# aukeschaap/ttcross

Hardware: AMD Instinct MI355X
Metric: fiber evals/s (neval / wall time of dtt_dmrgg), Ising C_64 n=51 r=32 piv=2 (d=63) (higher is better)
Workload: dtype f64; 1 GPU; Ising C_64 n=51 r=32 piv=2 (d=63); driver=test_crs_ising c 64 51 32 2, bond_groups=8, transport=none (single process), arith=exact, sweeps=16

## Files before the change

### include/ttx.h

```cpp
#ifndef TTX_H
#define TTX_H
#include <stdint.h>

#ifdef __cplusplus
extern "C" {
#endif

#define TTX_OK 0
#define TTX_EINVAL 1
#define TTX_ENODEV 2
#define TTX_EHIP 3
#define TTX_ESTATE 4

#define TTX_FUN_ISING 1
#define TTX_FUN_STDNORM 2
#define TTX_FUN_MVN 3
#define TTX_FUN_HOST 4
#define TTX_FUN_COSCOEFF 5
#define TTX_FUN_DEVICE 6
#define TTX_FUN_TRAINS 7
#define TTX_FUN_PULLBACK 8

#define TTX_ARITH_EXACT 0
#define TTX_ARITH_FAST 1
// ... 163 lines not shown
int ttx_cores_dot_dev  (ttx_engine *h, const double *a_dev, const double *b_dev, double *out );
int ttx_cores_axpby_dev(ttx_engine *h, double alpha, const double *x_dev, double beta, double *y_dev);
int ttx_cores_get      (ttx_engine *h, double *g);
int ttx_cores_set      (ttx_engine *h, const double *g);
int ttx_cores_get_dev  (ttx_engine *h, double *g_dev);
int ttx_cores_set_dev  (ttx_engine *h, const double *g_dev);
int ttx_basis_fit_batch    (ttx_engine *h, int64_t npts, const double *x, const ttx_basis *basis, const double *y, const double *w, const ttx_fit_opts *opts,
                            double *loss, double *lambda, int32_t *cg_iters, int32_t *accepted, ttx_fit_result *result);
int ttx_basis_fit_batch_dev(ttx_engine *h, int64_t npts, const double *x_dev, const ttx_basis *basis, const double *y_dev, const double *w_dev, const ttx_fit_opts *opts,
                            double *loss, double *lambda, int32_t *cg_iters, int32_t *accepted, ttx_fit_result *result);
int ttx_basis_fit_tab      (ttx_engine *h, int64_t npts, const double *phi, const double *y, const double *w, const ttx_fit_opts *opts,
                            double *loss, double *lambda, int32_t *cg_iters, int32_t *accepted, ttx_fit_result *result);
int ttx_basis_fit_tab_dev  (ttx_engine *h, int64_t npts, const double *phi_dev, const double *y_dev, const double *w_dev, const ttx_fit_opts *opts,
                            double *loss, double *lambda, int32_t *cg_iters, int32_t *accepted, ttx_fit_result *result);
int ttx_basis_fit_last     (const ttx_engine *h, double *ms_jvp, double *ms_core_grad, double *ms_value, double *ms_vector, int64_t *n_jvp, int64_t *n_core_grad, int32_t *mode_ran);

int ttx_sq_lognorm_grad     (ttx_engine *h, const double *const *md, const double *const *mo, double gvol, double coef, double *g, int32_t accumulate, int32_t mode, double *z_mant, int64_t *z_exp, double *logz);
int ttx_sq_lognorm_grad_dev (ttx_engine *h, const double *const *md, const double *const *mo, double gvol, double coef, double *g_dev, int32_t accumulate, int32_t mode, double *z_mant, int64_t *z_exp, double *logz);
int ttx_sq_lognorm_grad_last(const ttx_engine *h, double *ms_right, double *ms_left, double *ms_asm, double *flops, int32_t *mode_ran);
int ttx_sq_nll_batch    (ttx_engine *h, int64_t npts, const double *x , const ttx_basis *basis , const double *w, double gamma, const double *const *md, const double *const *mo,
                         double gvol, int32_t mode, double *nll, double *logz, double *val, double *g);
int ttx_sq_nll_batch_dev(ttx_engine *h, int64_t npts, const double *x_dev, const ttx_basis *basis, const double *w_dev, double gamma, const double *const *md, const double *const *mo,
                         double gvol, int32_t mode, double *nll, double *logz, double *val_dev, double *g_dev);

int ttx_sample(ttx_engine *h, int64_t npts, const double *u , const double *w, const int32_t *fixed, int32_t *ind, double *logq, double *val);
int ttx_sample_dev(ttx_engine *h, int64_t npts, const double *u, const double *w, const int32_t *fixed, int32_t *ind, double *logq, double *val);
int ttx_sample_last(const ttx_engine *h, double *ms_head, double *bytes_head, double *ms_draw, int64_t *nfailed);

int ttx_sample_sq    (ttx_engine *h, int64_t npts, const double *u , const double *w, const int32_t *fixed,
                      double gamma, int32_t mode, int32_t *ind, double *logq, double *val);
int ttx_sample_sq_dev(ttx_engine *h, int64_t npts, const double *u, const double *w, const int32_t *fixed,
                      double gamma, int32_t mode, int32_t *ind, double *logq, double *val);
int ttx_sample_sq_last(const ttx_engine *h, double *ms_head, double *ms_rows, double *ms_pick, double *flops, int64_t *nfailed, int32_t *mode_ran);

int ttx_sample_real    (ttx_engine *h, int64_t npts, const double *u , const double *const *nodes ,
                        const double *cond , double *x , int32_t *cell , double *logq, double *val);
int ttx_sample_real_dev(ttx_engine *h, int64_t npts, const double *u, const double *const *nodes, const double *cond, double *x, int32_t *cell, double *logq, double *val);
int ttx_sample_real_last(const ttx_engine *h, double *ms_head, double *bytes_head, double *ms_draw, int64_t *nfailed);

int ttx_sample_sq_real    (ttx_engine *h, int64_t npts, const double *u , const double *const *nodes ,
                           const double *cond , double gamma, int32_t mode, double *x , int32_t *cell ,
                           double *logq, double *val);
int ttx_sample_sq_real_dev(ttx_engine *h, int64_t npts, const double *u, const double *const *nodes, const double *cond, double gamma, int32_t mode, double *x,
                           int32_t *cell, double *logq, double *val);
int ttx_sample_sq_real_last(const ttx_engine *h, double *ms_head, double *ms_rows, double *ms_pick, double *flops, int64_t *nfailed, int32_t *mode_ran);

int ttx_rosenblatt_sq_real    (ttx_engine *h, int64_t npts, const double *x , const double *const *nodes ,
                               const double *cond , double gamma, int32_t mode, double *u , int32_t *cell ,
                               double *logq, double *val);
int ttx_rosenblatt_sq_real_dev(ttx_engine *h, int64_t npts, const double *x, const double *const *nodes, const double *cond, double gamma, int32_t mode, double *u,
                               int32_t *cell, double *logq, double *val);
int ttx_rosenblatt_sq_real_last(const ttx_engine *h, double *ms_head, double *ms_rows, double *ms_cdf, double *flops, int64_t *nfailed, int32_t *mode_ran);

#define TTX_TOPK_ABS 0
#define TTX_TOPK_MAX 1
#define TTX_TOPK_MIN 2
int ttx_topk(ttx_engine *h, int32_t K, int32_t which, const int32_t *fixed , int32_t mode,
             int32_t *nfound, int32_t *ind , double *val , double *bound);
int ttx_topk_last(const ttx_engine *h, double *ms_gram, double *ms_score, double *ms_select, double *flops, int32_t *mode_ran);

int ttx_replicate(ttx_engine *h, ttx_engine **out);

int ttx_from_tt(ttx_engine **out, int32_t d, const int32_t *n, const int32_t *r, const double *cores, int32_t device);
int ttx_write(const ttx_engine *h, const char *path);
int ttx_read(ttx_engine **out, const char *path, int32_t device);
int ttx_get_modes(const ttx_engine *h, int32_t *d, int32_t *n);
int ttx_write_hdf5(const ttx_engine *h, const char *path);
int ttx_read_hdf5(ttx_engine **out, const char *path, int32_t device);

#define TTX_K_LOTTERY 0
#define TTX_K_HALFSTEP 1
#define TTX_K_ACCEPT 2
#define TTX_K_EXCHANGE 3
#define TTX_K_QUAD 4
#define TTX_K_OTHER 5
#define TTX_K_NKINDS 6
int ttx_set_profile(ttx_engine *h, int on);
int ttx_sweep_path(const ttx_engine *h);
int ttx_plan_describe(const ttx_engine *h, char *buf, int64_t cap);
int ttx_cluster_eval(const ttx_engine *h);
int ttx_arith(const ttx_engine *h);
int ttx_cluster_fallbacks(const ttx_engine *h);
int ttx_cluster_entry(const ttx_engine *h, int64_t out[3]);
int ttx_sweep_gap(const ttx_engine *h, int32_t out[4]);
int ttx_det_fallbacks(const ttx_engine *h);
int ttx_fun_id(const ttx_engine *h);
int64_t ttx_resid_halfsteps(const ttx_engine *h);
int ttx_kernel_stats(const ttx_engine *h, int64_t launches[TTX_K_NKINDS], double ms[TTX_K_NKINDS], double bytes[TTX_K_NKINDS]);


int ttx_k_residual_argmax(int32_t device, int32_t m, int32_t r, const double *a, const double *F, const double *x,
                          double *b_out, int32_t *imax, double *bmax);
int ttx_k_residual_bench(int32_t device, int64_t m, int32_t r, int32_t iters, double *avg_ms, double *bytes);
int ttx_k_eval(int32_t device, int32_t fun_id, int32_t d, const int32_t *n, const double *par, int32_t npar,
               const double *aux, int32_t naux, int64_t npts, const int32_t *ind, double *out);
int ttx_k_eval_arith(int32_t device, int32_t fun_id, int32_t d, const int32_t *n, const double *par, int32_t npar,
                     const double *aux, int32_t naux, int64_t npts, const int32_t *ind, double *out, int32_t arith);
int ttx_k_lottery(int32_t device, int32_t npnt, int32_t m, int32_t n, int32_t nz, const int32_t *zcol,
                  const int32_t *zrow, uint64_t rngpos, int32_t *points );
int ttx_k_fast_block(int32_t device, int32_t fun_id, int32_t d, int32_t n, const double *par, int32_t npar, const double *aux, int32_t naux,
                     int32_t p, int32_t rL, const int32_t *Lidx, int32_t rR, const int32_t *Ridx, int32_t cap, int32_t chain,
                     int64_t npts, const int32_t *pts, double *near, double *dv, double *piv, double *lot, double *colf, double *rowf,
                     double *nfar, double *pnt);
int ttx_fast_tables(const ttx_engine *h, int32_t group, int32_t side, int32_t bond, int32_t cols, int32_t *info, int32_t *idx, double *near,
                    double *dv, double *piv);

int ttx_k_exp(int32_t device, int64_t n, const double *x, double *out);
int ttx_exp_host(int64_t n, const double *x, double *out);

int ttx_k_latency_probe(int32_t device, double out[5]);

int ttx_k_rccl_selftest(int32_t device, int64_t msg_bytes, int32_t nsum);

int ttx_k_xcc_map(int32_t device, int32_t nblocks, int32_t *out);

#ifdef __cplusplus
}
#endif
#endif
```

### ttcross_amd/csrc/ttx_addr.h

```cpp
#pragma once
#include <hip/hip_runtime.h>
#include "ttx_dev.h"

__device__ __forceinline__ double *core_ptr(const DevProb &P, double *base, int g, int p, int first)
{ return base + ((size_t)g * P.NC + (p - first)) * P.CS; }
__device__ __forceinline__ double *inv_ptr(const DevProb &P, int g, int s, int first)
{ return P.inv + ((size_t)g * P.NC + (s - first + 1)) * (size_t)P.RM * P.RM; }
__device__ __forceinline__ int *vip_ptr(const DevProb &P, int g, int s, int first)
{ return P.vip + ((size_t)g * P.NC + (s - first + 1)) * (size_t)4 * P.RM; }
__device__ __forceinline__ short *L_ptr(const DevProb &P, int g, int s, int first)
{ return P.L + ((size_t)g * P.NC + (s - first + 1)) * (size_t)P.d * P.RM; }
__device__ __forceinline__ short *R_ptr(const DevProb &P, int g, int s, int first)
{ return P.R + ((size_t)g * P.NC + (s - first)) * (size_t)P.d * P.RM; }
```

### ttcross_amd/csrc/ttx_cluster.h

```cpp
#pragma once
#include "ttx_fused.h"
#include "ttx_mvn.h"
#include "ttx_cluster_rules.h"

#define CB 256

struct ClD2 { double a, b; };
struct ClStrided {
    const char *p; size_t sb; unsigned at;
    __device__ __forceinline__ ClStrided(const double *base, size_t at_, size_t stride) : p((const char *)base), sb(8 * stride), at((unsigned)(8 * at_)) {}
    __device__ __forceinline__ double operator()() { const double v = *(const double *)(p + at); p += sb; return v; }
};

__device__ __forceinline__ double f_ising_c4p(int m, int A, const double *an, const double *aw, double s1n, double s1w,
                                              double s2n, double s2w, const double *bn, const double *bw,
                                              double pv, double pvk, double pw, double pwk)
{
    const int nb = m - A - 2;
    double v = pv, w = pw, vk = pvk, wk = pwk;
    auto vstep = [&](double xv) { vk = vk * xv; v = v + vk; };
    auto wstep = [&](double xv) { wk = wk * xv; w = w + wk; };
    vstep(s2n); vstep(s1n);
    chain8v<true>(an, A, vstep);
    wstep(s1n); wstep(s2n);
// ... 47 lines not shown
}
__device__ __forceinline__ void wave_argmax2(double &a, double &v, int &idx)
{
    const double amx = wave_max_key(a);
    const int key = (a == amx && idx != INT_MAX) ? ((idx << 1) | (signbit(v) ? 1 : 0)) : INT_MAX;
    const int kmin = wave_min_i(key);
    a = amx;
    if (kmin == INT_MAX) { idx = INT_MAX; v = 0.0; }
    else { idx = kmin >> 1; v = (kmin & 1) ? -amx : amx; }
}

__device__ __forceinline__ double f_ising_cfast(double xj, double wj, double xk, double wk, double pv, double pvk, double pw, double pwk,
                                                double SL, double WL, double SR, double WR)
{
    const double v = pv + pvk * xk * (1.0 + xj * (1.0 + SL));
    const double w = pw + pwk * xj * (1.0 + xk * (1.0 + SR));
    return 2.0 / (v * w) * ((WL * wj) * (wk * WR));
}

typedef unsigned int u4 __attribute__((ext_vector_type(4)));
struct ClRec { u4 a, b; };
static_assert(sizeof(ClRec) == sizeof(ClPart), "record buffers are sized as ClPart: [2][G][TTX_CLREC] u4 arg-max records, then as many running-maximum records");
__device__ __forceinline__ void st16(void *p, u4 v) { asm volatile("global_store_dwordx4 %0, %1, off sc1" :: "v"(p), "v"(v) : "memory"); }
__device__ __forceinline__ u4 ld16(const void *p)
{
    u4 v;
    asm volatile("global_load_dwordx4 %0, %1, off sc1\n\ts_waitcnt vmcnt(0)" : "=v"(v) : "v"(p) : "memory");
    return v;
}

__device__ __forceinline__ int xcc_id() { return (int)__builtin_amdgcn_s_getreg(((4 - 1) << 11) | 20) & 15; }

__device__ __forceinline__ bool cluster_sync(unsigned *ctr, unsigned target, int *abortflag, int *s_ok)
{
    asm volatile("s_waitcnt vmcnt(0)" ::: "memory");
    __syncthreads();
    if (threadIdx.x == 0) {
        int ok = 1;
        unsigned spins = 0;
        __hip_atomic_fetch_add(ctr, 1u, __ATOMIC_RELEASE, __HIP_MEMORY_SCOPE_AGENT);
        while (__hip_atomic_load(ctr, __ATOMIC_RELAXED, __HIP_MEMORY_SCOPE_AGENT) < target) {
            __builtin_amdgcn_s_sleep(1);
            if (++spins > (1u << 22)) { ok = 0; __hip_atomic_store(abortflag, 1, __ATOMIC_RELAXED, __HIP_MEMORY_SCOPE_SYSTEM); break; }
            if ((spins & 1023u) == 0 && __hip_atomic_load(abortflag, __ATOMIC_RELAXED, __HIP_MEMORY_SCOPE_SYSTEM)) { ok = 0; break; }
        }
        __atomic_thread_fence(__ATOMIC_ACQUIRE);
        *s_ok = ok;
    }
    __syncthreads();
    return *s_ok != 0;
}

#ifdef TTX_STAMPS
#define CST_DECL const bool t_me = (threadIdx.x == 0 && g == 0 && cb == 0); long long t_prev = wall_clock64()
#define CST(k) do { if (t_me) { long long t_now = wall_clock64(); gs.stamp[0][k] += t_now - t_prev; t_prev = t_now; } } while (0)
#define CST_END() do { if (t_me) gs.nstamp[0]++; } while (0)
#define CSE_DECL const int t_eb = (threadIdx.x == 0 && g == 0 && cb <= 1) ? cb : -1; long long t_eprev = wall_clock64()
#define CSE_MARK() do { if (t_eb >= 0) t_eprev = wall_clock64(); } while (0)
#define CSE(k) do { if (t_eb >= 0) { long long t_now = wall_clock64(); P.gs[0].stamp[1][8 * t_eb + (k)] += t_now - t_eprev; t_eprev = t_now; } } while (0)
#define CSE_END() do { if (t_eb == 0) P.gs[0].nstamp[1]++; } while (0)
#define WST(k) do { if (P.dbg && g == 0 && epoch == 8 && pp == 4 && lane == 0 && h < 8) P.dbg[((size_t)(h * 64 + cb * 4 + wv)) * 8 + (k)] = (long long)__builtin_readcyclecounter(); } while (0)
#else
#define WST(k)
#define CST_DECL
#define CST(k)
#define CST_END()
#define CSE_DECL
#define CSE_MARK()
#define CSE(k)
#define CSE_END()
#endif

#define CL_ZKEEP 1
#define CL_ZCARRY 2
#define CL_WORD 4
#define CL_POWTAB 8
#define CL_PACK2 16
static_assert(CL_POWTAB_N == CB, "one table entry per thread of a workgroup");
__device__ const ClPowTab cl_powtab = cl_make_powtab();
struct ClArgs { DevProb P; int dir, nsteps, NB, ldsinv, epoch, zkeep; };
__device__ __forceinline__ int *cl_zimage(const DevProb &P, int g, int nsteps)
{ return (int *)(P.cl_part + (size_t)2 * P.G * TTX_CLREC) + (size_t)g * cl_zimage_ints(nsteps, P.RM); }

template <bool CFAST, bool CPAD>
__global__ __launch_bounds__(CB) void k_sweep_cluster(DevProb P, int dir, int nsteps, int NB, int ldsinv, int epoch, int zkeep)
{
    extern __shared__ __align__(16) double dyn[];
    __shared__ int zc[128], zr[128], zcs[128], zrs[128], keepc[128], keepr[128];
    __shared__ int nzc, nzr, nsc, nsr, s_ok;
    __shared__ int slt[2][TTX_CLMAX + 1], wtab[TTX_CLMAX];
    __shared__ ttx_cdfseg segc[TTX_TABSEG], segr[TTX_TABSEG];
    __shared__ double sha[8], shv[8], shm[8]; __shared__ int shi[8];
    __shared__ double pLw[64], pLk[64], pRv[64], pRk[64];
    static_assert(!(CFAST && CPAD), "the closed form reads the rows in dimension order");
    constexpr int NFT = CFAST ? 64 : 1;
    __shared__ double fSL[NFT], fWL[NFT], fSR[NFT], fWR[NFT];
    __shared__ struct { int ii, jj, kk, qq, hcount, rc_k, rc_q, rr_i, rr_j; double pivot, amax, bytes_half; long long neval, n_resid; } s_rook;
    const int bid = blockIdx.x;
    const int g = (bid & 7) + 8 * (bid / (8 * NB)), cb = (bid >> 3) % NB;
    CSE_DECL;
    if (g >= P.G || P.ctl[0]) return;
    const int bpar = (epoch - 1) & 1;
    if (P.tail_side && epoch >= 2) {
        const TailRec &t0 = P.tailrec[(size_t)bpar * P.G];
        if (stop_rule(epoch - 1, P.maxrank, P.accuracy, t0.pivotmax, max_pos(t0.amax, P.gs[0].amax_bnd[bpar]), P.strk[epoch & 1]).ready) return;
    }
    if (P.cl_test_abort && P.cl_test_abort == epoch && g == 0 && cb == 0) {
        if (threadIdx.x == 0) { __hip_atomic_store(P.cl_abort, 1, __ATOMIC_RELAXED, __HIP_MEMORY_SCOPE_SYSTEM); P.ctl[0] = 1; }
        return;
    }
    const int tid = threadIdx.x, m = P.d, RM = P.RM, NM = P.NM;
    const int lane = tid & 63, wv = tid >> 6;
    GroupState &gs = P.gs[g];
    const int first = gs.first, last = gs.last, nbonds = last - first + 1;
    int *r = P.r + (size_t)g * (m + 2);
    const int VS = ((m + 7) & ~7) + 8;
    const int RS = 2 * VS + 2;
    const int n1m = P.n[1];
    const int SL = RM * ((NM + NB - 1) / NB + 1);
    unsigned *ctr = P.cl_ctr + g;
    unsigned nbar = (unsigned)(epoch - 1) * (unsigned)min(nsteps, nbonds);
    ClPart *part = P.cl_part;
    double *par = dyn;
    double *XL = par + ((P.npar + 1) & ~1);
    double *XR = XL + (size_t)RM * RS;
    double *acol = XR + (size_t)RM * RS;
    double *arow = acol + SL;
    double *resc = arow + SL;
    double *resr = resc + SL;
    double *xsc = resr + SL;
    double *xsr = xsc + ((RM + 1) & ~1);
    int *lot = (int *)(xsr + ((RM + 1) & ~1));
    double *GL = (double *)(lot + 4 * ((2 * RM + 2 * NM + 4 + 1) & ~1));
    double *GU = GL + (size_t)RM * RM;
    int *ZK = (int *)(ldsinv ? GU + (size_t)RM * RM : GL);
    int *ZN = ZK + (size_t)nsteps * 2 * RM;
    for (int x = tid; x < P.npar; x += CB) par[x] = P.par[x];
    if (cb == 0) {
        if (tid == 0) { gs.pivotmax = -1.0; gs.pivotmin = -1.0; }
        int *rr = P.rr + (size_t)g * (m + 2);
        for (int s = tid; s <= m; s += CB) rr[s] = r[s];
    }
    __syncthreads();
    CSE(0);
    if ((zkeep & CL_ZCARRY) && cl_lists_valid(gs.zk_epoch, epoch)) {
        const int *img = cl_zimage(P, g, nsteps);
        for (int x = tid; x < nbonds * 2 * RM; x += CB) ZK[x] = img[x];
        for (int x = tid; x < 2 * nbonds; x += CB) ZN[x] = img[(size_t)nsteps * 2 * RM + x];
        if (cb == 0 && tid == 0) gs.n_zload++;
        __syncthreads();
    } else if (zkeep & CL_ZKEEP) {
        int *TMP = (int *)XL;
        const int E = nbonds * 2 * RM;
        for (int x = tid; x < E; x += CB) {
            const int b = x / (2 * RM), side = (x / RM) & 1, u = x % RM, pb = first + b;
            if (u < r[pb]) { const int *vp = vip_ptr(P, g, pb, first) + 4 * u; TMP[x] = (vp[2 * side + 1] << 16) | vp[2 * side]; }
        }
        __syncthreads();
        for (int x = tid; x < E; x += CB) {
            const int b = x / (2 * RM), u = x % RM, nb_ = r[first + b];
            if (u < nb_) {
                const int *src = TMP + (x - u); const int a = src[u]; int ra = 0;
                for (int t = 0; t < nb_; t++) ra += (src[t] < a) || (src[t] == a && t < u);
                ZK[(x - u) + ra] = a;
            }
        }
        __syncthreads();
        for (int x = tid; x < E; x += CB) {
            const int b = x / (2 * RM), u = x % RM, nb_ = r[first + b];
            if (u < nb_) {
                const int *src = ZK + (x - u); int pc = 0;
                for (int t = 1; t <= u; t++) pc += (src[t] != src[t - 1]);
                const bool keep = (u == 0) || (src[u] != src[u - 1]);
                TMP[x] = keep ? pc : -1;
                if (u == nb_ - 1) ZN[x / RM] = pc + 1;
            }
        }
        __syncthreads();
        int mykey = 0, mypos = -1;
        for (int x0 = 0; x0 < E; x0 += CB) {
            const int x = x0 + tid;
            mypos = -1;
            if (x < E) { const int b = x / (2 * RM), u = x % RM; if (u < r[first + b]) { mypos = TMP[x]; mykey = ZK[x]; } }
            __syncthreads();
            if (mypos >= 0) ZK[(x - x % RM) + mypos] = mykey;
            __syncthreads();
        }
    }
    double amax = gs.amax, pivotmax = -1.0, pivotmin = -1.0;
    if (P.tail_side && epoch >= 2) amax = max_pos(amax, gs.amax_bnd[bpar]);
    const double pivotmax_prev = gs.pivotmax_prev;
    long long neval = gs.neval;
    unsigned long long rngpos = gs.rngpos;
    double bytes_half = gs.bytes_half; long long n_resid = gs.n_resid;
    int hcount = 0;
    CSE(1);
    const bool ptab = (zkeep & CL_POWTAB) != 0;
    const unsigned long long bil0 = ptab ? cl_powtab.v[tid] : ttx_minstd_pow(2ull * tid);
    unsigned long long sA0;
    {
        const unsigned long long cw = gs.rngword, cwpos = gs.rngword_pos;
        if ((zkeep & CL_WORD) && cl_word_valid(cw, cwpos, rngpos)) { sA0 = cw; if (cb == 0 && tid == 0) gs.n_wload++; }
        else sA0 = ttx_minstd_pow(2 * rngpos + 1);
    }
    const int bl0 = ptab ? (int)cl_powtab.v[lane] : (int)ttx_minstd_pow(2ull * lane);
    constexpr unsigned long long c64 = cl_minstd_pow_c(128);
    CSE(2);
    CST_DECL;

    for (int pp = 1; pp <= nsteps; pp++) {
        if (pp > nbonds) break;
        const int p = (dir == 1) ? first + pp - 1 : last + 1 - pp;
        const int r0 = r[p - 1], r1 = r[p], r2 = r[p + 1], n1 = P.n[p], n2 = P.n[p + 1];
        const int nlot = r0 + n1 + n2 + r2;
        double *Cp = core_ptr(P, P.col, g, p, first), *Wq = core_ptr(P, P.row, g, p + 1, first);
        double *Ap = core_ptr(P, P.arg, g, p, first), *Aq = core_ptr(P, P.arg, g, p + 1, first);
        const short *Lt = L_ptr(P, g, p - 1, first), *Rt = R_ptr(P, g, p + 1, first);
        const int cA = (p - 1 + 7) >> 3, cB = (m - p - 1 + 7) >> 3;
        const int sside = (tid >> 6) & 1, sseg = tid & 63;
        double sg_a0 = 0.0, sg_al = 0.0, sg_de = 0.0; int sg_k0 = 0, sg_cn = 0, myns = 0;
        auto seg_issue = [&](int Kc_, int Kr_) {
            if (tid >= 128) {
                const int K = sside ? Kr_ : Kc_; const ttx_cdfseg *sp = P.cdf_tab + (size_t)K * TTX_TABSEG + sseg;
                myns = P.cdf_ns[K]; sg_a0 = sp->a0; sg_al = sp->alast; sg_de = sp->delta; sg_k0 = sp->k0; sg_cn = sp->cnt;
            }
        };
        {
            const int AL = min(VS, (p - 1 + 7) & ~7), AR = min(VS, (m - p - 1 + 7) & ~7);
            if (AL > 0) {
                int c = tid / AL, o = tid - c * AL;
                const int dc = CB / AL, dO = CB - dc * AL;
                while (c < r0) {
                    if constexpr (CPAD) {
                        if (o < p - 1) {
                            const int ix = (int)Lt[(size_t)o * RM + c];
                            XL[(size_t)c * RS + (p - 2 - o)] = par[ix - 1]; XL[(size_t)c * RS + VS + o] = par[n1m + ix - 1];
                        } else { XL[(size_t)c * RS + o] = 0.0; XL[(size_t)c * RS + VS + o] = 1.0; }
                    } else {
                        const int ix = (o < p - 1) ? (int)Lt[(size_t)o * RM + c] : 1;
                        XL[(size_t)c * RS + o] = par[ix - 1]; XL[(size_t)c * RS + VS + o] = par[n1m + ix - 1];
                    }
                    c += dc; o += dO; if (o >= AL) { o -= AL; c++; }
                }
            }
            if (AR > 0) {
                int c = tid / AR, o = tid - c * AR;
                const int dc = CB / AR, dO = CB - dc * AR;
                while (c < r2) {
                    if (CPAD && o >= m - p - 1) { XR[(size_t)c * RS + o] = 0.0; XR[(size_t)c * RS + VS + o] = 1.0; }
                    else {
                        const int ix = (o < m - p - 1) ? (int)Rt[(size_t)o * RM + c] : 1;
                        XR[(size_t)c * RS + o] = par[ix - 1]; XR[(size_t)c * RS + VS + o] = par[n1m + ix - 1];
                    }
                    c += dc; o += dO; if (o >= AR) { o -= AR; c++; }
                }
            }
        }
        if (ldsinv) {
            if (p > first) { const double *gL = inv_ptr(P, g, p - 1, first); for (int x = tid; x < r0 * r0; x += CB) GL[x] = gL[x]; }
            if (p < last)  { const double *gU = inv_ptr(P, g, p + 1, first); for (int x = tid; x < r2 * r2; x += CB) GU[x] = gU[x]; }
        }
        CST(0);
        if (zkeep & CL_ZKEEP) seg_issue(r0 * n1 - ZN[2 * (p - first)], n2 * r2 - ZN[2 * (p - first) + 1]);
        static_assert(2 * (TTX_CLMAX + 1) <= 64 && TTX_CLMAX + TTX_CLMAX + 2 < 64, "the two slice rows and the shuffles of the fill fit one wave");
        if (wv == CB / 64 - 1) {
            const int side = lane > TTX_CLMAX ? 1 : 0, c = lane - side * (TTX_CLMAX + 1);
            const int s = cl_slice(min(c, NB), side ? n2 : n1, NB);
            const int s1 = __shfl(s, lane + 1), t0 = __shfl(s, lane + TTX_CLMAX + 1), t1 = __shfl(s, lane + TTX_CLMAX + 2);
            if (lane < 2 * (TTX_CLMAX + 1)) slt[side][c] = s;
            if (lane < TTX_CLMAX) wtab[lane] = cl_wact(s1 - s, t1 - t0, r0, r2, CB / 64);
        }
        if (tid == 0) s_ok = 1;
        const unsigned long long stepmul = cl_stepmul(nlot, [&](int b) { return (unsigned long long)(unsigned)__shfl(bl0, b); }, c64);
        const unsigned long long sA1 = ttx_mulmod31(sA0, stepmul);
        if (zkeep & CL_ZKEEP) {
            const int b = p - first;
            const int *kc = ZK + (size_t)b * 2 * RM, *kr = kc + RM;
            if (tid == 0) { nzc = ZN[2 * b]; nzr = ZN[2 * b + 1]; }
            if (tid < ZN[2 * b]) zc[tid] = ((kc[tid] & 0xffff) - 1) + r0 * ((kc[tid] >> 16) - 1) + 1;
            if (tid < ZN[2 * b + 1]) zr[tid] = ((kr[tid] & 0xffff) - 1) + n2 * ((kr[tid] >> 16) - 1) + 1;
            __syncthreads();
        } else bond_zero_lists(vip_ptr(P, g, p, first), r1, r0, n2, tid, zc, zr, zcs, zrs, keepc, keepr, &nzc, &nzr);
        CST(1);
        const int Kc = r0 * n1 - nzc, Kr = n2 * r2 - nzr;
        if (!(zkeep & CL_ZKEEP)) seg_issue(Kc, Kr);
        if (tid >= 128) {
            ttx_cdfseg *dst = sside ? segr : segc;
            if (sseg < myns) { dst[sseg].a0 = sg_a0; dst[sseg].alast = sg_al; dst[sseg].delta = sg_de; dst[sseg].k0 = sg_k0; dst[sseg].cnt = sg_cn; }
            if (sseg == 0) { if (sside) nsr = myns; else nsc = myns; }
        }
        if (tid < r0) {
            double w = 1.0, wk = 1.0;
            auto wstep = [&](double xv) { wk = wk * xv; w = w + wk; };
            if constexpr (CPAD) chain8v<true>(XL + (size_t)tid * RS, p - 1, wstep);
            else chain8v<false>(XL + (size_t)tid * RS, p - 1, wstep);
            pLw[tid] = w; pLk[tid] = wk;
            if constexpr (CFAST) {
                double sk = 1.0, ss = 0.0, ww = 1.0;
                auto sstep = [&](double xv) { sk = sk * xv; ss = ss + sk; };
                auto pstep = [&](double xv) { ww = ww * xv; };
                chain8v<true>(XL + (size_t)tid * RS, p - 1, sstep);
                chain8v<false>(XL + (size_t)tid * RS + VS, p - 1, pstep);
                fSL[tid] = ss; fWL[tid] = ww;
            }
        } else if (tid >= 64 && tid < 64 + r2) {
            const int c = tid - 64;
            double v = 1.0, vk = 1.0;
            auto vstep = [&](double xv) { vk = vk * xv; v = v + vk; };
            chain8v<true>(XR + (size_t)c * RS, m - p - 1, vstep);
            pRv[c] = v; pRk[c] = vk;
            if constexpr (CFAST) {
                double sk = 1.0, ss = 0.0, ww = 1.0;
                auto sstep = [&](double xv) { sk = sk * xv; ss = ss + sk; };
                auto pstep = [&](double xv) { ww = ww * xv; };
                chain8v<false>(XR + (size_t)c * RS, m - p - 1, sstep);
                chain8v<false>(XR + (size_t)c * RS + VS, m - p - 1, pstep);
                fSR[c] = ss; fWR[c] = ww;
            }
        }
        __syncthreads();
        CST(2);
        const int jlo = __builtin_amdgcn_readfirstlane(slt[0][cb]), jhi = __builtin_amdgcn_readfirstlane(slt[0][cb + 1]);
        const int klo = __builtin_amdgcn_readfirstlane(slt[1][cb]), khi = __builtin_amdgcn_readfirstlane(slt[1][cb + 1]);
        const int nj = jhi - jlo, nk = khi - klo;
        double ma = 0.0, ba = -1.0, bv = 0.0; int bi = INT_MAX;
        const int nscu = __builtin_amdgcn_readfirstlane(nsc), nsru = __builtin_amdgcn_readfirstlane(nsr);
        const int nzcu = __builtin_amdgcn_readfirstlane(nzc), nzru = __builtin_amdgcn_readfirstlane(nzr);
        const int r1u = __builtin_amdgcn_readfirstlane(r1);
        for (int il = tid; il < nlot; il += CB) {
            const unsigned long long bil = (il == tid) ? bil0 : ttx_minstd_pow(2ull * il);
            const double d1 = ttx_flang_from_word(ttx_mulmod31(sA0, bil)), d2 = ttx_flang_from_word(ttx_mulmod31(sA1, bil));
            const ttx_pair xy = ttx_lottery_index2<TTX_TABSEG, 64>(segc, nscu, Kc, r0 * n1, zc, nzcu, d1, segr, nsru, Kr, n2 * r2, zr, nzru, d2);
            const int x = xy.x, y = xy.y;
            CST(3);
            const int i = (x - 1) % r0 + 1, j = (x - 1) / r0 + 1, k = (y - 1) % n2 + 1, q = (y - 1) / n2 + 1;
            lot[4 * il] = i; lot[4 * il + 1] = j; lot[4 * il + 2] = k; lot[4 * il + 3] = q;
            const double *rl = XL + (size_t)(i - 1) * RS, *rq = XR + (size_t)(q - 1) * RS;
            double f;
            if constexpr (CFAST) f = f_ising_cfast(par[j - 1], par[n1m + j - 1], par[k - 1], par[n1m + k - 1], pRv[q - 1], pRk[q - 1], pLw[i - 1], pLk[i - 1], fSL[i - 1], fWL[i - 1], fSR[q - 1], fWR[q - 1]);
            else if constexpr (CPAD) f = f_ising_c4w(cA, cB, rl, rl + VS, par[j - 1], par[n1m + j - 1], par[k - 1], par[n1m + k - 1], rq, rq + VS, pRv[q - 1], pRk[q - 1], pLw[i - 1], pLk[i - 1]);
            else f = f_ising_c4p(m, p - 1, rl, rl + VS, par[j - 1], par[n1m + j - 1], par[k - 1], par[n1m + k - 1], rq, rq + VS, pRv[q - 1], pRk[q - 1], pLw[i - 1], pLk[i - 1]);
            ma = fmax(ma, fabs(f));
            CST(4);
            ClStrided lc(Cp, (i - 1) + (size_t)RM * (j - 1), P.SS), lw(Wq, (k - 1) + (size_t)NM * (q - 1), P.SW);
            double t = 0.0;
            cl_ordered_sum<8>(r1u, [&] { const double cv = lc(); return ClD2{cv, lw()}; }, [&](int, ClD2 e) { t = t + e.a * e.b; });
            const double b = f - t, aa = fabs(b);
            if (aa > ba || (aa == ba && il < bi)) { ba = aa; bv = b; bi = il; }
        }
        ma = wave_max_key(ma);
        wave_argmax2(ba, bv, bi);
        if (lane == 0) { shm[wv] = ma; sha[wv] = ba; shv[wv] = bv; shi[wv] = bi; }
        __syncthreads();
        ma = shm[0]; ba = sha[0]; bv = shv[0]; bi = shi[0];
        for (int x = 1; x < CB / 64; x++) {
            ma = fmax(ma, shm[x]);
            if (sha[x] > ba || (sha[x] == ba && shi[x] < bi)) { ba = sha[x]; bv = shv[x]; bi = shi[x]; }
        }
        amax = fmax(amax, ma);
        neval += nlot; rngpos += 2ull * nlot;
        sA0 = ttx_mulmod31(sA1, stepmul);
        if (bi == INT_MAX) bi = 0;
        int ii = lot[4 * bi], jj = lot[4 * bi + 1], kk = lot[4 * bi + 2], qq = lot[4 * bi + 3];
        double pivot = bv;
        CST(5);
        int havecol = 0, haverow = 0, crs = 0, done = 0;
        int rc_k = -1, rc_q = -1, rr_i = -1, rr_j = -1;
        const int H = (P.piv == 0) ? 2 : 2 * P.piv;
        double mxrun = 0.0;
        const bool rook_active = wv < wtab[cb];
        const bool slot_on = (lane < NB * (CB / 64)) && ((lane & (CB / 64 - 1)) < wtab[lane / (CB / 64)]);
        if (rook_active) {
        for (int h = 0; h < H && !done; h++) {
            const bool iscol = (P.piv == 0) ? (h == 0) : (((h + (dir == 2 ? 1 : 0)) & 1) == 0);
            const int nf = iscol ? r0 * n1 : n2 * r2;
            const int nsl = iscol ? r0 * nj : nk * r2;
            double *fib = iscol ? acol : arow;
            double xsv = 0.0;
            if (lane < r1) xsv = iscol ? Wq[(kk - 1) + (size_t)NM * (qq - 1) + P.SW * lane] : Cp[(ii - 1) + (size_t)RM * (jj - 1) + P.SS * lane];
            crs++;
            if (iscol) havecol = 1; else haverow = 1;
            const int dn = (P.piv == 0) ? (h == 1) : (havecol && haverow && (crs >= 2 * P.piv));
            const bool resid = (P.piv != 0) && !dn;
            if (iscol) { rc_k = resid ? kk : -1; rc_q = qq; } else { rr_i = resid ? ii : -1; rr_j = jj; }
            CST(6);
            WST(0);
            double mx = 0.0, ab = -1.0, bb = 0.0; int ix = INT_MAX;
            for (int u = tid; u < nsl; u += CB) {
                double a;
                if (iscol) {
                    const int i = u % r0, j = jlo + u / r0, t = i + r0 * j;
                    const double *rl = XL + (size_t)i * RS, *rq = XR + (size_t)(qq - 1) * RS;
                    if constexpr (CFAST) a = f_ising_cfast(par[j], par[n1m + j], par[kk - 1], par[n1m + kk - 1], pRv[qq - 1], pRk[qq - 1], pLw[i], pLk[i], fSL[i], fWL[i], fSR[qq - 1], fWR[qq - 1]);
// ... 38 lines not shown
            if (lane == 0) {
                const unsigned long long ua = (unsigned long long)__double_as_longlong(ab), um = (unsigned long long)__double_as_longlong(mxrun);
                u4 ra, rb;
                rb.x = (unsigned)um; rb.y = (unsigned)(um >> 32); rb.z = gen; rb.w = 0;
                st16(&bufB[cb * (CB / 64) + wv], rb);
                if (xchg) {
                    ra.x = (unsigned)ua; ra.y = (unsigned)(ua >> 32); ra.z = (unsigned)ix; ra.w = gen | (signbit(bb) ? 0x80000000u : 0u);
                    st16(&bufA[cb * (CB / 64) + wv], ra);
                }
            }
            CST(8);
            WST(3);
            int ok = 1;
            ab = -1.0; bb = 0.0; ix = INT_MAX;
            if (xchg && slot_on) {
                unsigned spins = 0;
                for (;;) {
                    const u4 ra = ld16(&bufA[lane]);
                    if ((ra.w & 0x7fffffffu) == gen) {
                        ab = __longlong_as_double((long long)(((unsigned long long)ra.y << 32) | ra.x));
                        ix = (int)ra.z;
                        bb = (ra.w & 0x80000000u) ? -ab : ab;
                        break;
                    }
                    if (++spins > 64u) __builtin_amdgcn_s_sleep(1);
                    if (spins > (1u << 22)) { ok = 0; break; }
                    if ((spins & 1023u) == 0 && __hip_atomic_load(P.cl_abort, __ATOMIC_RELAXED, __HIP_MEMORY_SCOPE_SYSTEM)) { ok = 0; break; }
                }
            }
            WST(4);
            ok = __all(ok);
            if (resid) wave_argmax2(ab, bb, ix);
            WST(5);
            if (!ok) {
                if (lane == 0) { __hip_atomic_store(P.cl_abort, 1, __ATOMIC_RELAXED, __HIP_MEMORY_SCOPE_SYSTEM); P.ctl[0] = 1; *(volatile int *)&s_ok = 0; }
                return;
            }
            CST(9);
            hcount++;
            neval += nf;
            bytes_half += resid ? 8.0 * ((double)nf * r1 + r1 + 2.0 * nf) : 8.0 * nf;
            n_resid += resid ? 1 : 0;
            done = dn;
            if (resid) {
                if (ix == INT_MAX) ix = 0;
                if (iscol) { const int i = ix % r0 + 1, j = ix / r0 + 1; done = havecol && haverow && (i == ii && j == jj); ii = i; jj = j; }
                else       { const int k = ix % n2 + 1, q = ix / n2 + 1; done = havecol && haverow && (k == kk && q == qq); kk = k; qq = q; }
                pivot = bb;
            }
        }
        if (P.piv != 0) {
            u4 *bufB = (u4 *)part + ((size_t)((hcount - 1) & 1) * P.G + g) * TTX_CLREC + (size_t)2 * P.G * TTX_CLREC;
            const unsigned gen = ((unsigned)epoch << 20) | (unsigned)hcount;
            double mx = 0.0; int ok = 1;
            if (slot_on) {
                unsigned spins = 0;
                for (;;) {
                    const u4 rb = ld16(&bufB[lane]);
                    if (rb.z == gen) { mx = __longlong_as_double((long long)(((unsigned long long)rb.y << 32) | rb.x)); break; }
                    if (++spins > 64u) __builtin_amdgcn_s_sleep(1);
                    if (spins > (1u << 22)) { ok = 0; break; }
                    if ((spins & 1023u) == 0 && __hip_atomic_load(P.cl_abort, __ATOMIC_RELAXED, __HIP_MEMORY_SCOPE_SYSTEM)) { ok = 0; break; }
                }
            }
            ok = __all(ok);
            if (!ok) {
                if (lane == 0) { __hip_atomic_store(P.cl_abort, 1, __ATOMIC_RELAXED, __HIP_MEMORY_SCOPE_SYSTEM); P.ctl[0] = 1; *(volatile int *)&s_ok = 0; }
                return;
            }
            amax = fmax(amax, wave_max_key(mx));
        }
        if (tid == 0) {
            s_rook.ii = ii; s_rook.jj = jj; s_rook.kk = kk; s_rook.qq = qq; s_rook.hcount = hcount; s_rook.rc_k = rc_k; s_rook.rc_q = rc_q;
            s_rook.rr_i = rr_i; s_rook.rr_j = rr_j; s_rook.pivot = pivot; s_rook.amax = amax; s_rook.bytes_half = bytes_half; s_rook.neval = neval; s_rook.n_resid = n_resid;
        }
        }
        __syncthreads();
        if (!*(volatile int *)&s_ok) return;
        if (!rook_active) {
            ii = s_rook.ii; jj = s_rook.jj; kk = s_rook.kk; qq = s_rook.qq; hcount = s_rook.hcount; rc_k = s_rook.rc_k; rc_q = s_rook.rc_q;
            rr_i = s_rook.rr_i; rr_j = s_rook.rr_j; pivot = s_rook.pivot; amax = s_rook.amax; bytes_half = s_rook.bytes_half; neval = s_rook.neval; n_resid = s_rook.n_resid;
        }
        CST(10);
        int *tape = P.tape + ((size_t)g * (m + 2) + p) * 4;
        const bool upd = accept_pivot(pivot, amax, pivotmax_prev, P.small_element, P.small_pivot);
        if (!upd) {
            if (cb == 0 && tid == 0) { tape[0] = tape[1] = tape[2] = tape[3] = -1; P.upd[(size_t)g * (m + 2) + p] = 0; }
        } else {
            const int i0 = ii - 1, j0 = jj - 1, k0 = kk - 1, q0 = qq - 1;
            double *gI = inv_ptr(P, g, p, first);
            const bool reuseA = (rc_k == kk && rc_q == qq), reuseB = (rr_i == ii && rr_j == jj);
            AppendTab tab{0, 0};
            if (cb == 0) tab = append_tables_fetch(P, g, p, first, ii, qq, tid);
            if (reuseA && reuseB) {
                if (cb == 0)
                    for (int s = tid; s < r1; s += CB) {
                        const double c = Wq[k0 + (size_t)NM * q0 + P.SW * s], w = Cp[i0 + (size_t)RM * j0 + P.SS * s];
                        gI[r1 * r1 + s] = w; gI[r1 * r1 + r1 + s] = c;
                    }
            } else {
                for (int s = tid; s < r1; s += CB) { xsc[s] = Wq[k0 + (size_t)NM * q0 + P.SW * s]; xsr[s] = Cp[i0 + (size_t)RM * j0 + P.SS * s]; }
                __syncthreads();
                if (cb == 0)
                    for (int s = tid; s < r1; s += CB) { gI[r1 * r1 + s] = xsr[s]; gI[r1 * r1 + r1 + s] = xsc[s]; }
            }
            for (int u = tid; u < r0 * nj; u += CB) {
                const int i = u % r0, j = jlo + u / r0; const size_t o = i + (size_t)RM * j;
                const double a = acol[u];
                Ap[o + P.SS * r1] = a;
                double y;
                if (reuseA) y = resc[u];
                else {
                    y = a;
                    ClStrided lc(Cp, o, P.SS); const double *xp = xsc;
                    cl_ordered_sum<16>(r1u, [&] { const double xv = *xp++; return ClD2{xv, lc()}; }, [&](int, ClD2 e) { y = y + (-e.a) * e.b; });
                }
                Cp[o + P.SS * r1] = (1.0 / pivot) * y;
            }
            for (int u = tid; u < nk * r2; u += CB) {
                const int k = klo + u % nk, q = u / nk;
                const double a = arow[u];
                Aq[r1 + (size_t)RM * k + P.SS * q] = a;
                const size_t o = k + (size_t)NM * q;
                if (reuseB) Wq[o + P.SW * r1] = resr[u];
                else {
                    double tt = 0.0;
                    ClStrided lw(Wq, o, P.SW); const double *xp = xsr;
                    cl_ordered_sum<16>(r1u, [&] { const double xv = *xp++; return ClD2{lw(), xv}; }, [&](int, ClD2 e) { tt = tt + e.a * e.b; });
                    Wq[o + P.SW * r1] = a + (-1.0) * tt;
                }
            }
            CST(11);
            if (p > first) {
                const double *gL = ldsinv ? GL : inv_ptr(P, g, p - 1, first);
                double *Wp = core_ptr(P, P.row, g, p, first);
                const int pk = (r0 <= 32) ? 2 : 1, lw = 64 / pk, l = lane & (lw - 1), sub = lane / lw;
                for (int base = wv * pk; base < nj; base += (CB / 64) * pk) {
                    const int jl = base + sub, j = jlo + jl;
                    const bool on = (jl < nj) && (l < r0);
                    const double a = on ? acol[l + r0 * jl] : 0.0;
                    const double xf = (pk == 2) ? dev_solve_L<2>(gL, r0, a, l, sub) : dev_solve_L<1>(gL, r0, a, l, 0);
                    if (on) Wp[j + (size_t)NM * r1 + P.SW * l] = xf;
                }
            }
            CST(12);
            if (p < last) {
                const double *gU = ldsinv ? GU : inv_ptr(P, g, p + 1, first);
                double *Cq = core_ptr(P, P.col, g, p + 1, first);
                const int pk = (r2 <= 32) ? 2 : 1, lw = 64 / pk, l = lane & (lw - 1), sub = lane / lw;
                const double rdg = dev_solve_rdg(gU, r2, l);
                for (int base = wv * pk; base < nk; base += (CB / 64) * pk) {
                    const int kl = base + sub, k = klo + kl;
                    const bool on = (kl < nk) && (l < r2);
                    const double y0 = on ? arow[kl + nk * l] : 0.0;
                    const double y = (pk == 2) ? dev_solve_U<2>(gU, r2, y0, rdg, l, sub) : dev_solve_U<1>(gU, r2, y0, rdg, l, 0);
                    if (on) Cq[r1 + (size_t)RM * k + P.SS * l] = y;
                }
            }
            CST(13);
            if (cb == 0) {
                append_tables_store(P, g, p, first, r1, ii, jj, kk, qq, tid, CB, tab);
                if (tid == 0) append_scalars(P, g, p, first, r1, ii, jj, kk, qq, pivot);
            }
            if ((zkeep & CL_ZKEEP) && wv < 2) {
                const int b = p - first;
                int *kl = ZK + (size_t)b * 2 * RM + (size_t)wv * RM;
                const int nl = ZN[2 * b + wv];
                const int key = wv == 0 ? ((jj << 16) | ii) : ((qq << 16) | kk);
                const int v = (lane < nl) ? kl[lane] : INT_MAX;
                const bool dup = __ballot(v == key) != 0ull;
                const int pos = __popcll(__ballot(v < key));
                if (!dup) {
                    if (lane < nl && v > key) kl[lane + 1] = v;
                    if (lane == 0) { kl[pos] = key; ZN[2 * b + wv] = nl + 1; }
                }
            }
            pivot_range(pivotmax, pivotmin, fabs(pivot));
        }
        CST(14);
        if (!cluster_sync(ctr, (++nbar) * (unsigned)NB, P.cl_abort, &s_ok)) { if (tid == 0) P.ctl[0] = 1; return; }
        CST(15);
        CST_END();
    }
    CSE_MARK();
    if (cb == 1) {
        const ClArgs *K = (const ClArgs *)__builtin_amdgcn_kernarg_segment_ptr();
        asm volatile("" : "+s"(K));
        if (cl_pack_block(CL_PACK_LEFT, K->NB, (K->zkeep & CL_PACK2) != 0) == 1) exch_pack_left(K->P, g);
        CSE(3);
    }
    if (cb == 0) {
        const ClArgs *K = (const ClArgs *)__builtin_amdgcn_kernarg_segment_ptr();
        asm volatile("" : "+s"(K));
        if (K->zkeep & CL_ZCARRY) {
            const int ns = K->nsteps, rm = K->P.RM;
            int *img = cl_zimage(K->P, g, ns);
            for (int x = tid; x < nbonds * 2 * rm; x += CB) img[x] = ZK[x];
            for (int x = tid; x < 2 * nbonds; x += CB) img[(size_t)ns * 2 * rm + x] = ZN[x];
        }
        if (tid == 0) {
            gs.amax = amax; gs.pivotmax = pivotmax; gs.pivotmin = pivotmin; gs.neval = neval; gs.rngpos = rngpos;
            gs.bytes_half = bytes_half; gs.n_resid = n_resid;
            if (K->zkeep & CL_WORD) { gs.rngword = sA0; gs.rngword_pos = rngpos; }
            if (K->zkeep & CL_ZCARRY) gs.zk_epoch = K->epoch;
            if (P.tail_side) gs.amax_bnd[epoch & 1] = 0.0;
        }
        __syncthreads();
        exch_pack_right(P, g);
        if (cl_pack_block(CL_PACK_LEFT, K->NB, (K->zkeep & CL_PACK2) != 0) == 0) exch_pack_left(P, g);
        CSE(3);
        CSE_END();
    }
}
```

### ttcross_amd/csrc/ttx_cluster_rules.h

```cpp
#pragma once
#include "ttx_cdf.h"

TTX_HD int cl_slice(int c, int n, int NB) { return (int)((unsigned)c * (unsigned)n / (unsigned)NB); }

TTX_HD int cl_wact(int nj, int nk, int r0, int r2, int nw)
{
    const int a = r0 * nj, b = nk * r2, e = a > b ? a : b, w = (e + 63) >> 6;
    return w < 1 ? 1 : (w > nw ? nw : w);
}

struct ClKey { int hi; unsigned lo; };
TTX_HD ClKey cl_key(double x) { const uint64_t b = ttx_dbits(x); return ClKey{(int)(uint32_t)(b >> 32), (unsigned)b}; }
TTX_HD double cl_unkey(ClKey k) { return ttx_bitsd(((uint64_t)(uint32_t)k.hi << 32) | k.lo); }
TTX_HD unsigned cl_key_lo_at(ClKey k, int hmax) { return k.hi == hmax ? k.lo : 0u; }

#if defined(__clang__)
#define CL_UNROLL _Pragma("unroll")
#define CL_NO_UNROLL _Pragma("unroll 1")
#else
#define CL_UNROLL
#define CL_NO_UNROLL
#endif
template <int N, class LD, class TM>
TTX_HD void cl_sum_piece(int s0, LD &ld, TM &tm)
{
    decltype(ld()) v[N];
    CL_UNROLL
    for (int k = 0; k < N; k++) v[k] = ld();
    CL_UNROLL
    for (int k = 0; k < N; k++) tm(s0 + k, v[k]);
}
template <int B, class LD, class TM>
TTX_HD void cl_ordered_sum(int n, LD ld, TM tm)
{
    static_assert(B == 16 || B == 8, "batches of 16 or 8 terms");
    int s = 0;
    CL_NO_UNROLL
    for (; s + B <= n; s += B) cl_sum_piece<B>(s, ld, tm);
    const int rem = n - s;
    if constexpr (B > 8) if (rem & 8) { cl_sum_piece<8>(s, ld, tm); s += 8; }
    if (rem & 4) { cl_sum_piece<4>(s, ld, tm); s += 4; }
    if (rem & 2) { cl_sum_piece<2>(s, ld, tm); s += 2; }
    if (rem & 1) cl_sum_piece<1>(s, ld, tm);
}

#define CL_POWTAB_N 256
constexpr uint64_t cl_mulmod31_c(uint64_t a, uint64_t b)
{
    uint64_t x = a * b;
    x = (x & 2147483647ULL) + (x >> 31);
    x = (x & 2147483647ULL) + (x >> 31);
    return (x >= 2147483647ULL) ? x - 2147483647ULL : x;
}
constexpr uint64_t cl_minstd_pow_c(uint64_t e)
{
    uint64_t base = 48271ULL, w = 1;
    while (e) { if (e & 1) w = cl_mulmod31_c(w, base); base = cl_mulmod31_c(base, base); e >>= 1; }
    return w;
}
struct ClPowTab { uint32_t v[CL_POWTAB_N]; };
constexpr ClPowTab cl_make_powtab()
{
    ClPowTab t{};
    for (int k = 0; k < CL_POWTAB_N; k++) t.v[k] = (uint32_t)cl_minstd_pow_c(2ULL * (uint64_t)k);
    return t;
}

template <class LANE>
TTX_HD uint64_t cl_stepmul(int nlot, LANE lane, uint64_t c64)
{
    if (nlot >= 512) return ttx_minstd_pow(2ull * (uint64_t)nlot);
    uint64_t s = lane(nlot & 63);
    for (int a = 0; a < (nlot >> 6); a++) s = ttx_mulmod31(s, c64);
    return s;
}

TTX_HD bool cl_word_valid(uint64_t word, uint64_t wpos, uint64_t rngpos) { return word != 0 && wpos == rngpos; }
TTX_HD bool cl_lists_valid(int tag, int epoch) { return tag != 0 && tag == epoch - 1; }
#define CL_PACK_RIGHT 0
#define CL_PACK_LEFT 1
TTX_HD int cl_pack_block(int part, int NB, bool split) { return (part == CL_PACK_LEFT && split && NB >= 2) ? 1 : 0; }
TTX_HD size_t cl_zimage_ints(int nsteps, int RM) { return ((size_t)nsteps * 2 * (size_t)RM + 2 * (size_t)nsteps + 3) & ~(size_t)3; }
```

### ttcross_amd/csrc/ttx_create_plan.h

```cpp
#pragma once
#include <algorithm>
#include <cmath>
#include <cstdarg>
#include <cstddef>
#include <cstdio>
#include <cstdlib>
#include <cstring>
#include <mutex>
#include <string>
#include <vector>

#include "../../include/ttx.h"
#include "ttx_dev.h"
#include "ttx_qr_plan.h"

#if defined(__HIPCC__)
#define TTX_PLAN_HD __host__ __device__ inline
#else
#define TTX_PLAN_HD inline
#endif

#define DE5_W 4
#define DE5_SEG 16
TTX_PLAN_HD size_t de5_lds_doubles(int m) { const int VS = ((m + 7) & ~7) + 8 + DE5_SEG; return (size_t)5 * VS + 128 + (size_t)DE5_W * 64; }
TTX_PLAN_HD bool de5_fits(int m) { return m >= 3; }
TTX_PLAN_HD int de_rows_stride(int m) { const int s = m + 56; return ((s + 31) & ~31) + 16; }
TTX_PLAN_HD size_t de_rows_lds_doubles(int m) { return (size_t)12 * de_rows_stride(m); }
TTX_PLAN_HD int det_vs(int m) { return ((m + 7) & ~7) + 8; }
TTX_PLAN_HD size_t det_lds_doubles(int m, int nbk) { return (size_t)4 * det_vs(m) + 256 + (det_vs(m) + 48) + (size_t)3 * nbk * 16 * 64; }

constexpr int TTX_PLAN_FB = 1024;
constexpr int TTX_PLAN_FNR = 24;
constexpr int TTX_PLAN_MVN_MAXQ = 8;

struct EnvText { bool set = false; std::string v; };
struct CreateEnv {
    EnvText arith;
    EnvText sweep;
    EnvText cl_pad;
    bool fullpiv_mfma = false;
    bool fast_persist_off = false;
    bool de_lane = false;
    bool de_tables_off = false, de_fastdiv_off = false, de_cut_off = false, de_v2_off = false, de_team_off = false;
    bool de_lot_point_set = false; int de_lot_point = 0;
    int de_team_units = 256, de_team6_units = 1024;
    int de_test_fault = 0;
    bool de_v5 = false;
    int cluster_nb = 8;
    bool cluster_coop = false;
    int cluster_test_abort = 0;
    bool dbg_waves = false;
    bool lottery_one_block = false;
    bool lottery_wave_off = false;
    bool lottery_rows2 = false;
    bool mvn_v2_off = false;
    bool tail_off = false;
    bool tail_side_off = false;
    bool head_direct_off = false;
    bool init_wave_off = false;
    bool fin_early_off = false;
    bool fin_skip_exch_off = false;
    bool init_wide_off = false;
    bool quad_lds_off = false;
    bool cl_powtab_off = false;
    bool cl_word_off = false;
    bool cl_lists_off = false;
    EnvText tail_event;
    bool tail_lean_off = false;
    bool cl_pack2_off = false;
};
template <class Get>
CreateEnv create_env_from(Get get)
{
    auto text = [&](const char *name) { EnvText t; if (const char *e = get(name)) { t.set = true; t.v = e; } return t; };
    auto num = [&](const char *name, int dflt) { const char *e = get(name); return e ? atoi(e) : dflt; };
    auto off = [&](const char *name) { const char *e = get(name); return e && atoi(e) == 0; };
    CreateEnv v;
    v.arith = text("TTX_ARITH"); v.sweep = text("TTX_SWEEP"); v.cl_pad = text("TTX_CL_PAD");
    v.fullpiv_mfma = text("TTX_FULLPIV").v == "mfma";
    v.fast_persist_off = off("TTX_FAST_PERSIST");
    v.de_lane = num("TTX_DE_LANE", 0) == 1;
    v.de_tables_off = off("TTX_DE_TABLES"); v.de_fastdiv_off = off("TTX_DE_FASTDIV"); v.de_cut_off = off("TTX_DE_CUT");
    v.de_v2_off = off("TTX_DE_V2"); v.de_team_off = off("TTX_DE_TEAM");
    v.de_lot_point_set = get("TTX_DE_LOT_POINT") != nullptr; v.de_lot_point = num("TTX_DE_LOT_POINT", 0);
    v.de_team_units = num("TTX_DE_TEAM_UNITS", v.de_team_units); v.de_team6_units = num("TTX_DE_TEAM6_UNITS", v.de_team6_units);
    v.de_test_fault = num("TTX_DE_TEST_FAULT", 0);
    v.de_v5 = num("TTX_DE_V5", 0) == 1;
    v.cluster_nb = num("TTX_CLUSTER_NB", v.cluster_nb);
    v.cluster_coop = num("TTX_CLUSTER_COOP", 0) == 1;
    v.cluster_test_abort = num("TTX_CLUSTER_TEST_ABORT", 0);
    v.dbg_waves = get("TTX_DBG_WAVES") != nullptr;
    v.lottery_one_block = num("TTX_LOTTERY_NB", 0) == 1;
    v.lottery_wave_off = off("TTX_LOTTERY_WAVE");
    v.lottery_rows2 = num("TTX_LOTTERY_ROWS", 0) == 2;
    v.mvn_v2_off = off("TTX_MVN_V2");
    v.tail_off = off("TTX_TAIL"); v.tail_side_off = off("TTX_TAIL_SIDE");
    v.head_direct_off = off("TTX_HEAD_DIRECT"); v.init_wave_off = off("TTX_INIT_WAVE");
    v.fin_early_off = off("TTX_FIN_EARLY"); v.fin_skip_exch_off = off("TTX_FIN_SKIP_EXCH");
    v.init_wide_off = off("TTX_INIT_WIDE"); v.quad_lds_off = off("TTX_QUAD_LDS");
    v.cl_powtab_off = off("TTX_CL_POWTAB"); v.cl_word_off = off("TTX_CL_WORD"); v.cl_lists_off = off("TTX_CL_LISTS");
    v.tail_event = text("TTX_TAIL_EVENT"); v.tail_lean_off = off("TTX_TAIL_LEAN");
    v.cl_pack2_off = off("TTX_CL_PACK2");
    return v;
}
struct DevCaps { int ncu = 0; bool coop = false; };

enum SweepWant { SWEEP_AUTO, SWEEP_CHAIN, SWEEP_FUSED, SWEEP_CLUSTER };
enum SlotKind { SLOTS_NONE, SLOTS_HOST, SLOTS_DEVICE };

struct CdfTables { std::vector<ttx_cdfseg> tab; std::vector<int> ns; };

struct CreatePlan {
    int err = TTX_OK; std::string errtext;
    int d = 0, RM = 0, NM = 0, W = 1, wrank = 0, nproc = 1, g0 = 0, G = 0, nbmax = 0, NC = 0, mode = 0, H = 0;
    std::vector<int32_t> own;
    int ising_id = 0; bool isDE = false;
    double mvn_norm = 1.0;
    size_t SS = 0, SW = 0, CS = 0, XD = 0, IOFF = 0, MSZ = 0, QB = 0, SB = 0, VS = 0;
    int nfb = 0, nlotmax = 0;
    int nn = 0, snum = 0;
    SlotKind slots = SLOTS_NONE; size_t HS = 0;
    int cdf_kmax = -1;
    bool pfull = false, qscr = false;
    bool want_fast = false;
    bool unit_nodes = false;
    int arith = 0, FD = 0, fpersist = 0;
    bool fast_tables = false;
    int de_npair = 0;
    int de_unit = 0, de_cut = 0;
    int de_slots = 0;
    int de_v2 = 0;
    int de_team = 0, de_team_units = 256, de_team6_units = 1024;
    int de_v5 = 0;
    int de_test_fault = 0;
    int de_lot_point = 0;
    int lot_wave = 0, lot_rows = 0;
    size_t lds_de = 0, lds_det = 0, lds_det6 = 0, lds_de5 = 0, lds_der = 0;
    int mvn_v2 = 0; size_t lds_mvn = 0;
    int lot_nb = 1, bnd_wave = 0;
    bool lot_cand = false;
    int fp_mfma = 0, fp_tiles = 0;
    size_t lds_par = 0, lds_half = 0, lds_lot = 0;
    int half_vals = 0, lot_vals = 0, fast_cap = 0;
    size_t lds_fused = 0, lds_cluster = 0;
    bool fused_ok = false;
    int cluster_cand = 0;
    int cluster_var = 0;
    int cluster_ldsinv = 0, cluster_zkeep = 0, cluster_coop = 0;
    bool cl_powtab = true, cl_word = true, cl_lists = false;
    int cl_test_abort = 0; bool dbg_waves = false;
    bool sweep_tail = true;
    bool sweep_tail_side = true;
    bool tail_event_kernel = true;
    bool tail_lean = true;
    bool cl_pack2 = true;
    bool head_direct = true;
    size_t lds_qtree = 0;
    bool init_wide = true;
    bool init_wave = true;
    bool fin_early = true;
    bool fin_skip_exch = true;
    SweepWant sweep_want = SWEEP_AUTO; int ncu = 0;
    int fused = 0;
    int cluster = 0;
};

inline size_t quad_tree_lds(int nproc, size_t RM, bool on)
{
    const size_t need = sizeof(double) * 2 * (size_t)nproc * RM * RM;
    return on && nproc > 1 && need <= TTX_LDS_WORK ? need : 0;
}
struct InitSamplesPlan { int threads = 256, rows = 0; size_t lds = 0; };
inline InitSamplesPlan init_samples_plan(size_t lds_par, size_t VS, int d, long nsamples, bool own_rows, bool wide)
{
    InitSamplesPlan p;
    const size_t lds1 = lds_par + 16 + sizeof(short) * 256 * VS;
    p.rows = lds1 <= TTX_LDS_WORK ? 1 : 0;
    p.lds = p.rows ? lds1 : lds_par;
    if (!p.rows || !wide || !own_rows) return p;
    const int threads = (int)std::min<long>(512, std::max<long>(256, (nsamples + 63) / 64 * 64));
    const size_t lds2 = lds_par + 16 + sizeof(short) * (size_t)threads * VS + 16 + sizeof(int) * (size_t)(d + 1);
    if (lds2 <= TTX_LDS_WORK) { p.threads = threads; p.rows = 2; p.lds = lds2; }
    return p;
}

inline void share(int first, int last, int nproc, std::vector<int32_t> &own)
{
    own.assign(nproc + 1, 0);
    own[0] = first;
    for (int p = 1; p < nproc; p++) own[p] = first + (int)((double)(last - first + 1) * (double)p / nproc);
    own[nproc] = last + 1;
}
inline double powi(double a, int b)
{
    double r = 1.0;
    for (;;) { if (b & 1) r *= a; b /= 2; if (b == 0) break; a *= a; }
    return r;
}
inline bool cdf_tables(int kmax, CdfTables &out)
{
    out.tab.assign((size_t)(kmax + 1) * TTX_TABSEG, ttx_cdfseg());
    out.ns.assign(kmax + 1, 0);
    std::vector<ttx_cdfseg> tmp(TTX_MAXSEG);
    for (int K = 1; K <= kmax; K++) {
        const int n_ = ttx_cdf_build(K, tmp.data());
        if (n_ > TTX_TABSEG) { out = CdfTables(); return false; }
        out.ns[K] = n_;
        memcpy(&out.tab[(size_t)K * TTX_TABSEG], tmp.data(), sizeof(ttx_cdfseg) * n_);
    }
    return true;
}
inline bool cdf_table_fits(int kmax)
{
    static std::mutex mu;
    static int looked = 0, first_over = -1;
    if (kmax > 16384) return false;
    std::lock_guard<std::mutex> lk(mu);
    std::vector<ttx_cdfseg> tmp(TTX_MAXSEG);
    while (looked < kmax && first_over < 0) { looked++; if (ttx_cdf_build(looked, tmp.data()) > TTX_TABSEG) first_over = looked; }
    return first_over < 0 || kmax < first_over;
}

#if defined(__GNUC__)
__attribute__((format(printf, 3, 4)))
#endif
inline CreatePlan &plan_refuse(CreatePlan &p, int code, const char *fmt, ...)
{
    char buf[512];
    va_list ap; va_start(ap, fmt); vsnprintf(buf, sizeof buf, fmt, ap); va_end(ap);
    p.err = code; p.errtext = buf;
    return p;
}
// ... 39 lines not shown
    p.QB = (size_t)nproc * RM * RM + 2 * nproc;
    p.lds_qtree = quad_tree_lds(nproc, RM, !env.quad_lds_off);
    p.SB = SUM_HDR + nproc + 5 * (size_t)(d + 1);
    p.qscr = 2 * sizeof(double) * (RM * RM + 2) > TTX_LDS_WORK;
    p.nn = cfg.n[0];
    for (int k = 1; k < d; k++) p.nn = std::min(p.nn, cfg.n[k]);
    p.snum = std::max(8, nproc);

    bool want = cfg.arith == TTX_ARITH_FAST;
    if (cfg.arith != TTX_ARITH_EXACT && cfg.arith != TTX_ARITH_FAST) return plan_refuse(p, TTX_EINVAL, "ttx_create: arith must be TTX_ARITH_EXACT or TTX_ARITH_FAST (got %d)", cfg.arith);
    if (env.arith.set) {
        if (env.arith.v == "fast") want = true;
        else if (env.arith.v != "exact") return plan_refuse(p, TTX_EINVAL, "TTX_ARITH must be exact or fast (got %s)", env.arith.v.c_str());
    }
    p.want_fast = want && !nofun;
    bool unit = fun == TTX_FUN_ISING;
    for (int j = 0; unit && j < std::min(NM, (int)cfg.npar); j++) unit = cfg.par[j] >= 0.0 && cfg.par[j] <= 1.0;
    p.unit_nodes = unit;
    p.arith = (p.want_fast && ((p.isDE && unit) || fun == TTX_FUN_MVN)) ? 1 : 0;
    if (p.arith) {
        p.fast_tables = true;
        p.FD = d + 1;
        p.fpersist = (fun == TTX_FUN_MVN && env.fast_persist_off) ? 0 : 1;
    }
    if (p.isDE && !p.arith && env.de_lane) p.de_unit = unit;
    if (p.isDE && !p.arith && !env.de_lane && !env.de_tables_off) {
        p.de_npair = d * (d + 1) / 2;
        p.de_unit = unit && !env.de_fastdiv_off;
        p.de_cut = (p.de_unit && !env.de_cut_off) ? 1 : 0;
        p.de_lot_point = (env.de_lot_point_set ? env.de_lot_point : (int)(d <= 160)) != 0;
        p.de_slots = (int)RM * ((NM + 63) / 64);
        p.lds_de = sizeof(double) * (5 * VS + 256) + (p.de_cut ? sizeof(int) * VS : 0);
        p.de_v2 = cfg.pivoting >= 0 && p.de_slots <= TTX_MAXPART && p.lds_de <= TTX_LDS_WORK && !env.de_v2_off;
        p.lds_det = sizeof(double) * det_lds_doubles(d, 3);
        p.lds_det6 = sizeof(double) * det_lds_doubles(d, 1);
        p.de_team = p.de_v2 && !p.de_cut && p.lds_det <= TTX_LDS_WORK && !env.de_team_off;
        p.de_team_units = env.de_team_units;
        p.de_team6_units = env.de_team6_units;
        p.de_test_fault = env.de_test_fault;
        p.lds_de5 = sizeof(double) * de5_lds_doubles(d);
        p.de_v5 = p.de_v2 && !p.de_cut && de5_fits(d) && p.lds_de5 <= TTX_LDS_WORK && env.de_v5;
    }
    p.pfull = cfg.pivoting < 0;
    if (cfg.pivoting < 0 && env.fullpiv_mfma && RM <= 64 && (long long)(RM * NM) * (long long)(RM * NM) < (1LL << 31)) {
        const size_t side = RM * NM;
        p.fp_mfma = 1; p.fp_tiles = (int)(((side + 63) / 64) * ((side + 63) / 64));
    }
    if (cdf_table_fits(p.RM * NM)) p.cdf_kmax = p.RM * NM;

    p.lds_par = sizeof(double) * (cfg.npar + 2);
    {
        const size_t base = sizeof(double) * (cfg.npar + RM + 4);
        const size_t idx_bytes = sizeof(short) * ((RM + 1) * VS + 16), val_bytes = sizeof(double) * ((RM + 1) * 2 * VS + 4);
        p.half_vals = (fun == TTX_FUN_ISING && p.ising_id == 1 && base + val_bytes <= TTX_LDS_VALUES) ? 1 : 0;
        p.lds_half = base + (p.half_vals ? val_bytes : idx_bytes);
        const size_t dif_bytes = sizeof(double) * ((RM + 1) * VS + 4);
        if (fun == TTX_FUN_MVN && base + dif_bytes <= TTX_LDS_HALF_DIFF) { p.half_vals = 1; p.lds_half = base + dif_bytes; }
        if (p.arith) p.lds_half = std::max(p.lds_half, base + sizeof(double) * ((size_t)std::max(p.FD, TTX_PLAN_FNR) + 4 + RM + 2));
    }
    const size_t lot_hdr = sizeof(double) * (cfg.npar + 4) + sizeof(int) * 4 * (nlotmax + 4);
    {
        p.lds_lot = lot_hdr + sizeof(short) * (2 * RM * VS + 16);
        const size_t lot_dif = lot_hdr + sizeof(double) * (2 * RM * VS + 4);
        if (fun == TTX_FUN_MVN && lot_dif <= TTX_LDS_LOTTERY) { p.lot_vals = 1; p.lds_lot = lot_dif; }
        if (p.arith && fun == TTX_FUN_ISING) {
            const size_t hdr = lot_hdr + 32;
            const size_t rowb = 2 * sizeof(double) * RM;
            p.fast_cap = (int)std::min<size_t>(std::min<size_t>(40, (size_t)d + 1), hdr < TTX_LDS_VALUES ? (TTX_LDS_VALUES - hdr) / rowb : 0);
            p.lds_lot = std::max(p.lds_lot, hdr + rowb * p.fast_cap);
        }
    }
    {
        const bool fastc = fun == TTX_FUN_ISING && p.ising_id == 1 && cfg.pivoting >= 0 && p.cdf_kmax >= 0;
        p.lds_fused = sizeof(double) * (cfg.npar + 4 + 4 * RM * VS + 2 * RM * NM + RM + 4) + sizeof(int) * 4 * (nlotmax + 4);
        p.fused_ok = fastc && p.RM <= 64 && nlotmax <= TTX_PLAN_FB && p.lds_fused <= TTX_LDS_WORK;
        int NB = std::max(1, std::min(env.cluster_nb, TTX_CLMAX));
        while (NB > 1 && p.G * NB > caps.ncu / 2) NB--;
        const size_t SL = RM * ((NM + NB - 1) / NB + 1);
        p.lds_cluster = sizeof(double) * (cfg.npar + 4 + 2 * RM * (2 * VS + 2) + 4 * SL + 2 * RM + 8) + sizeof(int) * 4 * (nlotmax + 4);
        if (p.lds_cluster + sizeof(double) * 2 * RM * RM <= TTX_LDS_WORK) { p.cluster_ldsinv = 1; p.lds_cluster += sizeof(double) * 2 * RM * RM; }
        const size_t zk = sizeof(int) * ((size_t)p.nbmax * 2 * RM + 2 * p.nbmax + 4);
        if (p.lds_cluster + zk <= TTX_LDS_WORK) { p.cluster_zkeep = 1; p.lds_cluster += zk; }
        p.cl_powtab = !env.cl_powtab_off; p.cl_word = !env.cl_word_off; p.cl_lists = p.cluster_zkeep && !env.cl_lists_off;
        const bool cfastc = p.want_fast && fun == TTX_FUN_ISING && p.ising_id == 1;
        if (env.cl_pad.set && env.cl_pad.v != "0" && env.cl_pad.v != "1") return plan_refuse(p, TTX_EINVAL, "TTX_CL_PAD must be 0 or 1 (got %s)", env.cl_pad.v.c_str());
        p.cluster_var = cfastc ? 2 : (unit && !(env.cl_pad.set && env.cl_pad.v == "0")) ? 1 : 0;
        if (fastc && p.RM <= 64 && NB >= 2 && p.G * NB <= caps.ncu && p.lds_cluster <= TTX_LDS_WORK) {
            p.cluster_cand = NB;
            p.cluster_coop = caps.coop && env.cluster_coop;
        }
        p.cl_test_abort = env.cluster_test_abort; p.dbg_waves = env.dbg_waves;
        p.sweep_tail = !env.tail_off; p.sweep_tail_side = !env.tail_side_off;
        if (env.tail_event.set && env.tail_event.v != "marker" && env.tail_event.v != "kernel")
            return plan_refuse(p, TTX_EINVAL, "TTX_TAIL_EVENT must be marker or kernel (got %s)", env.tail_event.v.c_str());
        p.tail_event_kernel = !(env.tail_event.set && env.tail_event.v == "marker");
        p.tail_lean = !env.tail_lean_off; p.cl_pack2 = !env.cl_pack2_off;
        p.head_direct = !env.head_direct_off; p.init_wave = !env.init_wave_off; p.init_wide = !env.init_wide_off;
        p.fin_early = !env.fin_early_off; p.fin_skip_exch = !env.fin_skip_exch_off;
        const std::string want_sweep = env.sweep.set ? env.sweep.v : "auto";
        if (want_sweep == "cluster") p.sweep_want = SWEEP_CLUSTER;
        else if (want_sweep == "fused") p.sweep_want = SWEEP_FUSED;
        else if (want_sweep == "auto") p.sweep_want = SWEEP_AUTO;
        else if (want_sweep == "chain") p.sweep_want = SWEEP_CHAIN;
        else return plan_refuse(p, TTX_EINVAL, "TTX_SWEEP must be auto, chain, fused or cluster (got %s)", want_sweep.c_str());
    }
    if (!nofun && (p.lds_half > TTX_LDS_DEVICE || p.lds_lot > TTX_LDS_LOTTERY)) return plan_refuse(p, TTX_EINVAL, "problem too large for LDS staging (d*maxrank)");
    {
        const bool heavy = p.isDE || fun == TTX_FUN_MVN;
        if (heavy && !env.lottery_one_block) p.lot_nb = std::min((nlotmax + 63) / 64, 64);
        if (p.lot_nb > 1 && (nlotmax + p.lot_nb - 1) / p.lot_nb > 64) p.lot_nb = 1;
        if (fun == TTX_FUN_MVN && d <= 64 * TTX_PLAN_MVN_MAXQ && cfg.pivoting >= 0 && (int)RM * ((NM + 63) / 64) <= TTX_MAXPART && !env.mvn_v2_off) {
            p.lot_cand = true;
            p.mvn_v2 = 1; p.de_slots = (int)RM * ((NM + 63) / 64);
            p.bnd_wave = 1;
            p.lds_mvn = sizeof(double) * (3 * (size_t)d + 8);
        }
        if (p.isDE && p.arith) p.bnd_wave = 1;
        if (p.isDE && p.de_npair) {
            p.lot_cand = true;
            p.lds_der = sizeof(double) * de_rows_lds_doubles(d);
            p.lot_wave = p.de_v2 && !p.de_cut && p.lds_der <= TTX_LDS_WORK && !env.lottery_wave_off;
            p.bnd_wave = p.lot_wave || (p.de_cut && p.de_v2 && p.lds_der <= TTX_LDS_WORK);
            p.lot_rows = p.lot_wave ? (env.lottery_rows2 ? 2 : 1) : 0;
        }
    }
    if (fun == TTX_FUN_HOST || fun == TTX_FUN_COSCOEFF || fun == TTX_FUN_DEVICE || fun == TTX_FUN_TRAINS || fun == TTX_FUN_PULLBACK) {
        p.HS = std::max<size_t>({RM * NM, (size_t)p.nn * p.snum, (size_t)p.NC * NM, (size_t)nlotmax, (size_t)2 * NM, (size_t)256});
        p.slots = fun == TTX_FUN_HOST ? SLOTS_HOST : SLOTS_DEVICE;
    }
    return p;
}

inline void create_admit(CreatePlan &p, int occ)
{
    bool cluster_ok = p.cluster_cand != 0;
    if (cluster_ok) {
        const long long cap = (long long)occ * p.ncu;
        const long long grid = 8LL * p.cluster_cand * ((p.G + 7) / 8);
        if (grid * 2 > cap) cluster_ok = false;
    }
    if (p.sweep_want == SWEEP_CLUSTER) { if (cluster_ok) p.cluster = p.cluster_cand; }
    else if (p.sweep_want == SWEEP_FUSED) { if (p.fused_ok) p.fused = 1; }
    else if (p.sweep_want == SWEEP_AUTO) { if (cluster_ok) p.cluster = p.cluster_cand; else if (p.fused_ok && p.G == 1) p.fused = 1; }
    if (p.cluster && p.cluster_var == 2) p.arith = 1;
}
```

### ttcross_amd/csrc/ttx_dev.h

```cpp
#pragma once
#include <stdint.h>
#include "ttx_cdf.h"
#define TTX_TABSEG 64

#define TTX_MAXH 24
#define TTX_MAXPART 512
#define TTX_BLK 256
#define TTX_FS 8
#define XH 8
#define SUM_NEVAL 0
#define SUM_AMAX 1
#define SUM_PMAX 2
#define SUM_PMIN 3
#define SUM_BYTES 4
#define SUM_NRESID 5
#define SUM_VAL 6
#define SUM_HDR 8

struct StepState {
    int active;
    int p, r0, r1, r2, n1, n2;
    int ii, jj, kk, qq;
    int done, havecol, haverow, crs;
    int pending;
    int npart;
    double pivot;
};

struct Partial {
    double absmax;
    double val;
    int idx;
    int pad;
};

struct GroupState {
    int first, last;
    int gglobal;
    int pad0;
    double amax, pivotmax, pivotmin, pivotmax_prev;
    long long neval;
    unsigned long long rngpos;
    double val;
    double initval;
    double bytes_half;
    long long n_resid;
    double amax_bnd[2];
    unsigned long long rngword, rngword_pos;
    int zk_epoch, n_zload, n_wload, pad1;
#ifdef TTX_STAMPS
    long long stamp[2][16]; long long nstamp[2];
#endif
    StepState S[TTX_MAXH];
    Partial Pt[2][TTX_MAXPART];
};

struct LotPart { double ab, bv, ma; int il, i, j, k, q, pad; };

#define TTX_CLMAX 16
#define TTX_CLREC (4 * TTX_CLMAX)
struct ClPart { double ab, bb, mx; int ix, pad; };

struct TailRec { double amax, pivotmax, pivotmin, bytes_half, initval; long long neval, n_resid; };

struct DevProb {
    int d, RM, NM, G, NC;
    int fun_id, piv, npar, ising_id;
    int arith;
    double *fNear[2], *fDv[2], *fPiv[2];
    int FD;
    int fpersist;
    const double *auxS;
    int nprocs;
    int has_quad;
    double mvn_norm;
    double small_element, small_pivot;
    size_t SS, SW, CS;
    const int *n;
    const double *par;
    const double *aux;
    double *deTL, *deUL, *deTR;
    int de_npair;
    int de_unit;
    int de_cut;
    int *deCL, *deCR;
    const double *auxT;
    const double *quadw;
    double *arg, *col, *row;
    double *inv;
    int *vip;
    short *L, *R;
    int *r, *rr, *upd, *tape;
    double *acol, *arow;
    double *Tq;
    int *ind0;
    char *msgR, *msgL;
    char **inL, **inR;
    size_t MSZ, IOFF, XD;
    double *red;
    double *redsend, *redrecv;
    double *qsend, *qall;
    double *qwork;
    double *qscr;
    double *sumsend, *sumrecv;
    int g0;
    Partial *pfull;
    double *sb; Partial *pfull2; int fp_mfma, fp_tiles;
    int nfb;
    const ttx_cdfseg *cdf_tab;
    const int *cdf_ns;
    int cdf_kmax;
    GroupState *gs;
    int *ctl;
    int *rq;
    double accuracy; int maxrank;
    int tail_side;
    TailRec *tailrec; int *tail_tape; int *strk;
    struct LotPart *lotp;
    unsigned *lot_ctr;
    int lot_nb;
    int *lotc; double *lotf; int lot_max;
    int bnd_wave;
    int hostpass, HS;
    int slot_dev;
    int zbase;
    short *hidx;
    double *hval;
    unsigned char *hreq;
    unsigned *cl_ctr;
    int *cl_abort;
    int cl_test_abort;
    struct ClPart *cl_part;
    long long *dbg;
};

#ifdef TTX_STAMPS
#define STAMP_DECL const bool t_me = (threadIdx.x == 0 && blockIdx.x == 0 && blockIdx.y == 0); long long t_prev = wall_clock64(); int t_slot = 0
#define STAMP(gs, k) do { __syncthreads(); if (t_me) { long long t_now = wall_clock64(); (gs).stamp[k][t_slot++] += t_now - t_prev; t_prev = t_now; } } while (0)
#define STAMP_END(gs, k) do { if (t_me) (gs).nstamp[k]++; } while (0)
#else
#define STAMP_DECL
#define STAMP(gs, k)
#define STAMP_END(gs, k)
#endif
#define FUN_ISING 1
#define FUN_STDNORM 2
#define FUN_MVN 3
#define FUN_HOST 4
```

### ttcross_amd/csrc/ttx_engine.hip

```cpp
#include <hip/hip_runtime.h>
#include <hip/hip_ext.h>

#include <chrono>
#include <cmath>
#include <cstdarg>
#include <cstdio>
#include <cstdlib>
#include <cstring>
#include <map>
#include <memory>
#include <string>
#include <thread>
#include <type_traits>
#include <vector>

#include <atomic>
#include <dlfcn.h>
#include <rccl/rccl.h>

#include "../../include/ttx.h"
#include "../../include/ttx_device_fun.h"
#include "ttx_err.h"
#include "ttx_lds.h"
#include "ttx_qr_plan.h"
// ... 461 lines not shown
    if (!h->aux.empty()) A_(dev_upload(h, &daux, h->aux.data(), h->aux.size()));
    if (cfg.quadw) {
        h->quadw.assign((size_t)(d + 1) * NM, 0.0);
        size_t off = 0;
        for (int k = 1; k <= d; k++) { for (int j = 0; j < h->n1[k]; j++) h->quadw[(size_t)k * NM + j] = cfg.quadw[off + j]; off += h->n1[k]; }
        A_(dev_upload(h, &dq, h->quadw.data(), h->quadw.size()));
    }
    P.n = dn; P.par = dpar; P.aux = daux; P.quadw = dq;
    return TTX_OK;
}
static int create_integrand_tables(ttx_engine *h)
{
    const CreatePlan &s = h->sel;
    DevProb &P = h->P;
    const int d = s.d;
    const size_t G = s.G, NC = s.NC, RM = s.RM;
    const bool mvn = h->cfg.fun_id == TTX_FUN_MVN;
    if (s.fast_tables) {
        const size_t slots = s.fpersist ? G * NC : G;
        for (int sd = 0; sd < 2; sd++) {
            A_(dev_alloc(h, &P.fNear[sd], slots * (size_t)s.FD * RM));
            A_(dev_alloc(h, &P.fPiv[sd], slots * (size_t)TTX_FS * RM));
            if (mvn) A_(dev_alloc(h, &P.fDv[sd], slots * (size_t)s.FD * RM));
        }
        if (mvn) {
            std::vector<double> sy((size_t)d * d);
            const double *ic = h->aux.data() + d;
            for (int i = 0; i < d; i++) for (int j = 0; j < d; j++) sy[i + (size_t)d * j] = 0.5 * (ic[i + (size_t)d * j] + ic[j + (size_t)d * i]);
            double *ds;
            A_(dev_upload(h, &ds, sy.data(), sy.size()));
            P.auxS = ds;
        }
    }
    if (s.de_npair) {
        A_(dev_alloc(h, &P.deTL, G * (size_t)s.de_npair * RM)); A_(dev_alloc(h, &P.deTR, G * (size_t)s.de_npair * RM));
        A_(dev_alloc(h, &P.deUL, G * (size_t)(d + 1) * RM));
        if (s.de_cut) { A_(dev_alloc(h, &P.deCL, G * (size_t)(d + 1) * RM)); A_(dev_alloc(h, &P.deCR, G * (size_t)(d + 1) * RM)); }
    }
    if (mvn) {
        std::vector<double> t((size_t)d * d);
        for (int i = 0; i < d; i++) for (int j = 0; j < d; j++) t[j + (size_t)d * i] = h->aux[d + i + (size_t)d * j];
        double *dt;
        A_(dev_upload(h, &dt, t.data(), t.size()));
        P.auxT = dt;
    }
    return TTX_OK;
}
static int create_cores(ttx_engine *h)
{
    const CreatePlan &s = h->sel;
    DevProb &P = h->P;
    const size_t d = s.d, G = s.G, NC = s.NC, RM = s.RM, NM = s.NM;
    A_(dev_alloc(h, &P.arg, G * NC * P.CS)); A_(dev_alloc(h, &P.col, G * NC * P.CS)); A_(dev_alloc(h, &P.row, G * NC * P.CS));
    A_(dev_alloc(h, &P.inv, G * NC * RM * RM)); A_(dev_alloc(h, &P.vip, G * NC * 4 * RM));
    A_(dev_alloc(h, &P.L, G * NC * d * RM)); A_(dev_alloc(h, &P.R, G * NC * d * RM));
    A_(dev_alloc(h, &P.r, G * (d + 2))); A_(dev_alloc(h, &P.rr, G * (d + 2))); A_(dev_alloc(h, &P.upd, G * (d + 2))); A_(dev_alloc(h, &P.tape, G * (d + 2) * 4));
    A_(dev_alloc(h, &P.acol, G * RM * NM)); A_(dev_alloc(h, &P.arow, G * RM * NM));
    A_(dev_alloc(h, &P.Tq, G * NC * RM * RM));
    A_(dev_alloc(h, &P.ind0, d + 2)); A_(dev_alloc(h, &P.gs, G));
    for (size_t g = 0; g < G; g++) {
        GroupState g0s{};
        g0s.first = h->own[h->g0 + g]; g0s.last = h->own[h->g0 + g + 1] - 1; g0s.gglobal = h->g0 + (int)g;
        const hipError_t e = hipMemcpy(P.gs + g, &g0s, offsetof(GroupState, S), hipMemcpyHostToDevice);
        if (e != hipSuccess) return fail(TTX_EHIP, "ttx_create: %s", hipGetErrorString(e));
    }
    if (s.pfull) A_(dev_alloc(h, &P.pfull, G * NM * RM * (size_t)s.nfb));
    if (s.fp_mfma) { A_(dev_alloc(h, &P.sb, G * (RM * NM) * (RM * NM))); A_(dev_alloc(h, &P.pfull2, G * (size_t)s.fp_tiles)); }
    if (s.cdf_kmax >= 0) {
        CdfTables t;
        if (!cdf_tables(s.cdf_kmax, t)) return fail(TTX_EINVAL, "ttx_create: no CDF tables up to K = %d", s.cdf_kmax);
        ttx_cdfseg *dt; int *dn_;
        A_(dev_upload(h, &dt, t.tab.data(), t.tab.size()));
        A_(dev_upload(h, &dn_, t.ns.data(), t.ns.size()));
        P.cdf_tab = dt; P.cdf_ns = dn_; P.cdf_kmax = s.cdf_kmax;
    }
    LotPart *lp; unsigned *lc;
    A_(dev_alloc(h, &lp, G * s.lot_nb));
    A_(dev_alloc(h, &lc, G));
    P.lotp = lp; P.lot_ctr = lc;
    if (s.lot_cand) { A_(dev_alloc(h, &P.lotc, G * s.nlotmax * 4)); A_(dev_alloc(h, &P.lotf, G * s.nlotmax)); }
    if (s.cluster) {
        unsigned *ctr; ClPart *cp;
        A_(dev_alloc(h, &ctr, G));
        A_(dev_alloc(h, &cp, 2 * G * TTX_CLREC + (s.cl_lists ? (G * cl_zimage_ints(s.nbmax, s.RM) * sizeof(int) + sizeof(ClPart) - 1) / sizeof(ClPart) : 0)));
        P.cl_ctr = ctr; P.cl_part = cp;
#ifdef TTX_STAMPS
        if (s.dbg_waves) { long long *dbg; A_(dev_alloc(h, &dbg, (size_t)8 * 64 * 8)); P.dbg = dbg; }
#endif
        HIPCHECK(hipHostMalloc((void **)&h->h_abort, sizeof(int)));
        *h->h_abort = 0;
        P.cl_abort = h->h_abort;
        P.cl_test_abort = s.cl_test_abort;
    }
    return TTX_OK;
}
static int create_exchange(ttx_engine *h)
{
    const CreatePlan &s = h->sel;
    DevProb &P = h->P;
    const size_t G = s.G, RM = s.RM, d = s.d;
    const int nproc = s.nproc;
    A_(dev_alloc(h, &P.msgR, G * P.MSZ)); A_(dev_alloc(h, &P.msgL, G * P.MSZ));
    A_(dev_alloc(h, &h->recvL, P.MSZ)); A_(dev_alloc(h, &h->recvR, P.MSZ));
    A_(dev_alloc(h, &P.inL, G)); A_(dev_alloc(h, &P.inR, G));
    A_(dev_alloc(h, &P.red, G * 4)); A_(dev_alloc(h, &P.redsend, 4));
    A_(dev_alloc(h, &P.qsend, h->QB)); A_(dev_alloc(h, &P.qwork, ((size_t)nproc + 2) * RM * RM)); A_(dev_alloc(h, &P.sumsend, h->SB));
    P.qscr = nullptr;
    if (s.qscr) A_(dev_alloc(h, &P.qscr, G * 2 * RM * RM));
    if (s.W > 1) { A_(dev_alloc(h, &P.redrecv, 4)); A_(dev_alloc(h, &P.qall, h->QB)); A_(dev_alloc(h, &P.sumrecv, h->SB)); }
    else { P.redrecv = P.redsend; P.qall = P.qsend; P.sumrecv = P.sumsend; }
    {
        std::vector<char *> il(G, nullptr), ir(G, nullptr);
        for (size_t g = 0; g < G; g++) {
            if (g > 0) il[g] = P.msgR + (g - 1) * P.MSZ; else if (h->g0 > 0) il[g] = h->recvL;
            if (g + 1 < G) ir[g] = P.msgL + (g + 1) * P.MSZ; else if (h->g0 + (int)G < nproc) ir[g] = h->recvR;
        }
        HIPCHECK(hipMemcpy(P.inL, il.data(), sizeof(char *) * G, hipMemcpyHostToDevice));
        HIPCHECK(hipMemcpy(P.inR, ir.data(), sizeof(char *) * G, hipMemcpyHostToDevice));
    }
    int *ctl, *rq;
    A_(dev_alloc(h, &ctl, (size_t)4));
    A_(dev_alloc(h, &rq, G * (d + 2)));
    P.ctl = ctl; P.rq = rq;
    P.tail_side = 0;
    A_(dev_alloc(h, &P.tailrec, 2 * G)); A_(dev_alloc(h, &P.tail_tape, 2 * G * (d + 2) * 4)); A_(dev_alloc(h, &P.strk, (size_t)2));
    return TTX_OK;
}
static int create_staging(ttx_engine *h)
{
    HIPCHECK(hipHostMalloc((void **)&h->h_sum_base, sizeof(double) * 2 * h->SB));
    h->h_sum = h->h_sum_base;
    memset(h->h_sum_base, 0, sizeof(double) * 2 * h->SB);
    HIPCHECK(hipHostMalloc((void **)&h->h_val, sizeof(double) * 2));
    HIPCHECK(hipStreamCreateWithFlags(&h->qstream, hipStreamNonBlocking));
    if (h->sel.lds_qtree) if (int rc = ensure_lds(h, reinterpret_cast<const void *>(k_quad_tree), h->sel.lds_qtree)) return rc;
    for (int x = 0; x < 2; x++) { HIPCHECK(hipEventCreateWithFlags(&h->ev_sum[x], hipEventDisableTiming)); HIPCHECK(hipEventCreateWithFlags(&h->ev_val[x], hipEventDisableTiming)); HIPCHECK(hipEventCreateWithFlags(&h->ev_tail[x], hipEventDisableTiming)); HIPCHECK(hipEventCreateWithFlags(&h->ev_qb[x], hipEventDisableTiming)); HIPCHECK(hipEventCreateWithFlags(&h->ev_fin[x], hipEventDisableTiming)); }
    HIPCHECK(hipHostMalloc((void **)&h->h_msg, 4 * h->P.MSZ));
    HIPCHECK(hipHostMalloc((void **)&h->h_tmp, sizeof(double) * std::max(h->QB, h->SB)));
    if (h->W > 1) {
        h->red_cap = std::max<size_t>(std::max(h->QB, h->SB), 8);
        HIPCHECK(hipHostMalloc((void **)&h->red_mem, sizeof(double) * h->red_cap * ttx_engine::NRED));
    }
    return TTX_OK;
}
static int create_slots(ttx_engine *h)
{
    const CreatePlan &s = h->sel;
    DevProb &P = h->P;
    if (s.slots == SLOTS_NONE) return TTX_OK;
    const size_t nslot = (size_t)s.G * s.HS, d = s.d;
    if (s.slots == SLOTS_DEVICE) {
        P.slot_dev = 1;
        A_(dev_alloc(h, &P.hidx, nslot * d)); A_(dev_alloc(h, &P.hval, nslot)); A_(dev_alloc(h, &P.hreq, nslot));
    } else {
        HIPCHECK(hipHostMalloc((void **)&P.hidx, sizeof(short) * nslot * d));
        HIPCHECK(hipHostMalloc((void **)&P.hval, sizeof(double) * nslot));
        HIPCHECK(hipHostMalloc((void **)&P.hreq, nslot));
        memset(P.hreq, 0, nslot); memset(P.hval, 0, sizeof(double) * nslot);
    }
    P.HS = (int)s.HS; P.hostpass = 0;
    return TTX_OK;
}
#undef A_

static int create_impl(ttx_engine **out, const ttx_config *cfg, bool nofun)
{
    if (!out || !cfg) return fail(TTX_EINVAL, "ttx_create: null argument");
    *out = nullptr;
// ... 609 lines not shown
        }
    }
    GroupState g0s;
    HIPCHECK(hipMemcpy(&g0s, P.gs, sizeof(GroupState), hipMemcpyDeviceToHost));
    for (int k = 0; k < 2; k++) {
        fprintf(stderr, "stamps kernel %d (n=%lld):", k, g0s.nstamp[k]);
        for (int x = 0; x < 16; x++) fprintf(stderr, " %.2fus", g0s.nstamp[k] ? 0.01 * (double)g0s.stamp[k][x] / (double)g0s.nstamp[k] : 0.0);
        fprintf(stderr, "\n");
    }
    return TTX_OK;
}
#endif

template <int FUN>
struct SweepRun {
    using clk = std::chrono::steady_clock;
    ttx_engine *const h; DevProb &P; const hipStream_t st;
    const int d, G, nproc, cluster, fused;
    const clk::time_point t0 = clk::now();
    LoopPlan L; ChainPlan plan;
    DevProb Pq;
    double val = 1.0, val_prev = 1.0;
    int strike = 0, sweeps = 0; bool ready = false, fin_enqueued = false;
    double *sum_final = nullptr;
    explicit SweepRun(ttx_engine *h_) : h(h_), P(h_->P), st(h_->stream), d(h_->d), G(h_->G), nproc(h_->cfg.nproc), cluster(h_->cluster_nb()), fused(h_->sel.fused) {}
    double since() const { return std::chrono::duration<double>(clk::now() - t0).count(); }
    template <class... A>
    int EV(const KLaunch &k, A... a)
    {
        if (FUN != FUN_HOST) { launch(st, k, P, a...); return TTX_OK; }
        DevProb Q = P;
        Q.hostpass = 1; launch(st, k, Q, a...);
        if (int rc = slot_eval(h)) return rc;
        Q.hostpass = 2; launch(st, k, Q, a...);
        return TTX_OK;
    }
    int prepare()
    {
        LoopIn in;
        in.whole = cluster || fused; in.cluster = cluster != 0; in.profile = h->profile; in.pipeline_off = env_off("TTX_PIPELINE");
        in.W = h->W; in.nproc = nproc; in.has_quad = P.has_quad; in.host_pass = FUN == FUN_HOST;
        in.sweep_tail = h->sel.sweep_tail; in.sweep_tail_side = h->sel.sweep_tail_side; in.maxrank = h->cfg.maxrank;
        in.head_direct = h->sel.head_direct; in.fin_early = h->sel.fin_early; in.fin_skip_exch = h->sel.fin_skip_exch;
        L = loop_plan(in);
        P.tail_side = L.side ? 1 : 0;
        h->recs.clear(); h->tapes.clear();
        plan = chain_plan<FUN>(h);
        for (const KLaunch *k : plan.all()) if (k->raise) if (int rc = ensure_lds(h, k->fn, k->lds)) return rc;
        if (fused) if (int rc = ensure_lds(h, reinterpret_cast<const void *>(k_sweep_fused), h->sel.lds_fused)) return rc;
        if (cluster) { if (int rc = ensure_lds_cluster(h)) return rc; *h->h_abort = 0; }
        Pq = P;
        if (L.pipe) Pq.r = P.rq;
        hipLaunchKernelGGL(k_reset, dim3(64), dim3(256), 0, st, P, h->SB, h->QB);
        {
            KScope ks(h, TTX_K_OTHER, 4);
            if (int rc = EV(plan.init_samples, h->sel.snum, h->sel.nn, FUN == FUN_HOST ? 0 : plan.srows, 0)) return rc;
            if (int rc = EV(plan.init_fibers)) return rc;
            hipLaunchKernelGGL(k_init_factors, dim3(h->NC, G), dim3(256), lds_fpersist(P), st, P);
            hipLaunchKernelGGL(k_init_final, dim3(G), dim3(256), 0, st, P, h->sel.init_wave ? 1 : 0, L.head_direct ? h->h_sum_base : (double *)nullptr);
        }
        if (L.head) {
            h->h_sum = h->h_sum_base;
            if (!L.head_direct) {
                hipLaunchKernelGGL(k_collect, dim3(1), dim3(256), 0, st, P);
                HIPCHECK(hipMemcpyAsync(h->h_sum, P.sumrecv, sizeof(double) * h->SB, hipMemcpyDeviceToHost, st));
            }
            HIPCHECK(hipEventRecord(h->ev_sum[0], st));
            if (int rc = launch_sweep_kernel(1)) return rc;
            HIPCHECK(hipEventSynchronize(h->ev_sum[0]));
        } else if (int rc = readback(h)) return rc;
        HIPCHECK(hipGetLastError());
        for (int g = 0; g < nproc; g++) val = (g == 0) ? h->h_sum[SUM_HDR + g] : val * h->h_sum[SUM_HDR + g];
        if (!P.has_quad) val = 0.0;
        val_prev = val;
        record(0, 0);
        ready = (1 >= h->cfg.maxrank);
        return TTX_OK;
    }
    int launch_sweep_kernel(int it_)
    {
        const CreatePlan &s = h->sel;
        int dir = 2 - it_ % 2, epoch = it_, nsteps = h->nbmax, NB = s.cluster, ldsinv = s.cluster_ldsinv;
        int zkeep = (s.cluster_zkeep ? CL_ZKEEP : 0) | (s.cl_lists ? CL_ZCARRY : 0) | (s.cl_word ? CL_WORD : 0) | (s.cl_powtab ? CL_POWTAB : 0)
                    | (s.cl_pack2 ? CL_PACK2 : 0);
        const dim3 grid(8 * NB * ((G + 7) / 8)), block(CB);
        KScope ks(h, TTX_K_HALFSTEP, 1);
        if (!cluster) hipLaunchKernelGGL(k_sweep_fused, dim3(G), dim3(FB), s.lds_fused, st, P, dir, nsteps);
        else if (s.cluster_coop) {
            void *args[] = {&P, &dir, &nsteps, &NB, &ldsinv, &epoch, &zkeep};
            HIPCHECK(hipLaunchCooperativeKernel(reinterpret_cast<const void *>(cluster_kernel(s.cluster_var)), grid, block, args, (unsigned)s.lds_cluster, st));
        } else hipLaunchKernelGGL(cluster_kernel(s.cluster_var), grid, block, s.lds_cluster, st, P, dir, nsteps, NB, ldsinv, epoch, zkeep);
        return TTX_OK;
    }
    int enqueue_chain_sweep(int it_)
    {
        const int dir = 2 - it_ % 2;
        const int rb = std::min((int)h->RM, it_ + 1);
        const int units = (h->sel.de_test_fault && it_ == h->sel.de_test_fault) ? 1 : rb * ((h->NM + 63) / 64);
        KLaunch half = plan.half[plan.ntier - 1].k;
        for (int t = plan.ntier - 2; t >= 0; t--) if (units * G <= plan.half[t].upto) { half = plan.half[t].k; half.grid.x = units; }
        for (int pp = 1; pp <= h->nbmax; pp++) {
            if (plan.tables) { KScope ks(h, TTX_K_OTHER); launch(st, plan.tables, P, dir, pp); }
            if (h->cfg.pivoting < 0) { if (int rc = enqueue_full_pivoting(dir, pp, rb)) return rc; }
            else {
                if (plan.lot_eval) {
                    KScope ks(h, TTX_K_LOTTERY, 3);
                    launch(st, plan.lottery, P, dir, pp, plan.lot_vals, 1);
                    launch(st, plan.lot_eval, P);
                    launch(st, plan.lottery, P, dir, pp, plan.lot_vals, 2);
                } else { KScope ks(h, TTX_K_LOTTERY); if (int rc = EV(plan.lottery, dir, pp, plan.lot_vals, 0)) return rc; }
                KScope ks(h, TTX_K_HALFSTEP, h->H);
                for (int hh = 0; hh < h->H; hh++) {
                    if (plan.half_vals < 0) launch(st, half, P, hh, dir, h->mode);
                    else if (int rc = EV(half, hh, dir, h->mode, plan.half_vals)) return rc;
                }
            }
            { KScope ks(h, TTX_K_ACCEPT); launch(st, plan.accept, P, h->H, plan.nfb); }
        }
        return TTX_OK;
    }
    int enqueue_full_pivoting(int dir, int pp, int rb)
    {
        KScope ks(h, TTX_K_HALFSTEP, 5);
        KLaunch cols = plan.base;
        cols.grid.z = h->NM * h->RM;
        hipLaunchKernelGGL(k_bond_begin, dim3(G), dim3(64), 0, st, P, dir, pp);
        if (plan.fullpiv == ChainPlan::FP_MFMA) {
            const int side = h->RM * h->NM, gx = (side + 63) / 64;
            launch(st, cols, P, 0, dir, 4, plan.base_vals);
            hipLaunchKernelGGL(k_full_gemm_argmax, dim3(gx, gx, G), dim3(256), 0, st, P);
            hipLaunchKernelGGL(k_full_resolve2, dim3(G), dim3(256), 0, st, P, gx, gx);
        } else if (plan.fullpiv == ChainPlan::FP_COLUMNS) {
            for (int z = 0; z < h->NM * rb; z++) {
                DevProb Q = P;
                Q.zbase = z;
                Q.hostpass = 1; launch(st, plan.base, Q, 0, dir, 3, 0);
                if (int rc = slot_eval(h)) return rc;
                Q.hostpass = 2; launch(st, plan.base, Q, 0, dir, 3, 0);
            }
            hipLaunchKernelGGL(k_full_resolve, dim3(G), dim3(256), 0, st, P);
        } else {
            launch(st, cols, P, 0, dir, 3, plan.base_vals);
            hipLaunchKernelGGL(k_full_resolve, dim3(G), dim3(256), 0, st, P);
        }
        if (int rc = EV(plan.base, 0, dir, 2, plan.base_vals)) return rc;
        return EV(plan.base, 1, dir, 2, plan.base_vals);
    }
    int enqueue_sweep_end(int it_)
    {
        const int slot = it_ & 1;
        if (L.side) return end_side(it_);
        if (L.forkq) HIPCHECK(hipStreamWaitEvent(st, h->ev_val[slot ^ 1], 0));
        if (int rc = L.tail ? end_tail(it_) : end_classic(it_)) return rc;
        if (L.pipe) HIPCHECK(hipEventRecord(h->ev_sum[slot], st));
        if (!P.has_quad) return TTX_OK;
        if (L.forkq) HIPCHECK(hipStreamWaitEvent(h->qstream, h->ev_sum[slot], 0));
        return enqueue_quadrature(it_, L.forkq ? h->qstream : st);
    }
    int tail_lean() const { return h->sel.tail_lean ? 1 : 0; }
    int end_side(int it_)
    {
        const int slot = it_ & 1;
        HIPCHECK(hipStreamWaitEvent(st, h->ev_val[slot ^ 1], 0));
        KScope ks(h, TTX_K_EXCHANGE, 1);
        if (h->sel.tail_event_kernel && !h->tail_event_retired) {
            const KLaunch &k = plan.exch_tail;
            int lean = tail_lean();
// ... 1315 lines not shown
        if (int rc = with_tier(s.tier, [&](auto mr) {
                constexpr int MR = decltype(mr)::value;
                if (int rc = op_lds_raise(h, reinterpret_cast<const void *>(k_ev_gemm<MR>), s.lds)) return rc;
                hipLaunchKernelGGL(k_ev_gemm<MR>, dim3(pl.g_gemm(i, c)), dim3(256), s.lds.bytes, h->stream, T, i, s.nmode, (const int *)off, (const int *)tile, (const int *)perm,
                                   (const double *)X, Z);
                return (int)TTX_OK;
            })) return rc;
        std::swap(X, Z);
    }
    hipLaunchKernelGGL(k_ev_final, dim3(pl.g_final(c)), dim3(256), 0, h->stream, c, T.ldx, (const int *)valid, (const double *)X, out);
    return TTX_OK;
}
extern "C" int ttx_eval_last_mode(const ttx_engine *h) { return h ? h->ev_last_mode : -1; }

static int ev_batch(ttx_engine *h, const char *who, EvStage st, int64_t npts, int32_t dd, const void *in, double *out, int32_t mode)
{
    int rc = tt_prepare(h, st == EV_HOST_COORD ? "dtt_value" : "dtt_ijk");
    if (rc) return rc;
    if (npts < 0 || (npts > 0 && (!in || !out))) return fail(TTX_EINVAL, "%s: null argument or negative npts", who);
    if (st == EV_HOST_COORD && dd < 1) return fail(TTX_EINVAL, "%s: %d coordinates per point", who, dd);
    if (!op_mode_known(mode)) return fail(TTX_EINVAL, "%s: unknown mode %d", who, mode);
    const EvPlan pl = ev_plan(h, st, npts, dd, mode);
    if (npts == 0) { if (st != EV_HOST_COORD) h->ev_last_mode = pl.eff; return TTX_OK; }
    const int32_t *ind = (const int32_t *)in;
    const double *x = (const double *)in;
    if (st == EV_HOST_COORD)
        for (size_t e = 0; e < (size_t)npts * dd; e++) if (!(x[e] < 2147483648.0)) return fail(TTX_EINVAL, "%s: coordinate %g of point %lld is not below 2^31", who, x[e], (long long)(e / dd));
    EvTrain T;
    if ((rc = ev_train(h, &T)) ||
        (rc = buf_reserve(h, {{SC_IND, pl.b_ind}, {SC_OUT, pl.b_out}, {SC_FLAG, pl.b_flag}, {SC_X, pl.b_x}, {SC_XA, pl.b_xa}, {SC_XB, pl.b_xb}, {SC_SORT, pl.b_sort}}))) return rc;
    const size_t d = h->d;
    int *sind = buf<int>(h, SC_IND), *sflag = st == EV_HOST_COORD ? buf<int>(h, SC_FLAG) : nullptr;
    double *sout = buf<double>(h, SC_OUT), *sx = buf<double>(h, SC_X);
    for (int64_t o = 0; o < npts; o += (int64_t)pl.chunk) {
        const int c = (int)std::min<int64_t>((int64_t)pl.chunk, npts - o);
        if (st == EV_ON_DEVICE) {
            if ((rc = ev_run(h, pl, T, c, ind + (size_t)o * d, nullptr, out + o))) return rc;
            continue;
        }
        if (st == EV_HOST_INDEX) HIPCHECK(hipMemcpyAsync(sind, ind + (size_t)o * d, sizeof(int) * (size_t)c * d, hipMemcpyHostToDevice, h->stream));
        else {
            HIPCHECK(hipMemcpyAsync(sx, x + (size_t)o * dd, sizeof(double) * (size_t)c * dd, hipMemcpyHostToDevice, h->stream));
            hipLaunchKernelGGL(k_ev_digits, g1((size_t)c), dim3(256), 0, h->stream, (int)d, T.n, (int)dd, (long long)c, (const double *)sx, sind, sflag);
        }
        if ((rc = ev_run(h, pl, T, c, sind, sflag, sout))) return rc;
        HIPCHECK(hipMemcpyAsync(out + o, sout, sizeof(double) * c, hipMemcpyDeviceToHost, h->stream));
        HIPCHECK(hipStreamSynchronize(h->stream));
    }
    if (st == EV_ON_DEVICE) HIPCHECK(hipStreamSynchronize(h->stream));
    HIPCHECK(hipGetLastError());
    h->ev_last_mode = pl.eff;
    return TTX_OK;
}
extern "C" int ttx_ijk_batch_dev(ttx_engine *h, int64_t npts, const int32_t *ind_dev, double *out_dev, int32_t mode)
{
    return ev_batch(h, "ttx_ijk_batch_dev", EV_ON_DEVICE, npts, 0, ind_dev, out_dev, mode);
}
extern "C" int ttx_ijk_batch(ttx_engine *h, int64_t npts, const int32_t *ind, double *out, int32_t mode)
{
    return ev_batch(h, "ttx_ijk_batch", EV_HOST_INDEX, npts, 0, ind, out, mode);
}
extern "C" int ttx_value_batch(ttx_engine *h, int64_t npts, int32_t dd, const double *x, double *out, int32_t mode)
{
    return ev_batch(h, "ttx_value_batch", EV_HOST_COORD, npts, dd, x, out, mode);
}

extern "C" int ttx_arith(const ttx_engine *h) { return h ? h->arith() : -1; }
extern "C" int ttx_sweep_path(const ttx_engine *h) { return !h ? -1 : h->cluster_nb() ? 2 : h->sel.fused ? 1 : 0; }
extern "C" int64_t ttx_resid_halfsteps(const ttx_engine *h) { return h ? h->n_resid : 0; }
extern "C" int ttx_cluster_eval(const ttx_engine *h) { return !h ? -1 : h->cluster_nb() ? 1 + h->sel.cluster_var : 0; }
extern "C" int ttx_cluster_fallbacks(const ttx_engine *h) { return h ? h->cluster_fallbacks : 0; }
extern "C" int ttx_cluster_entry(const ttx_engine *h, int64_t out[3])
{
    if (!h || !out) return fail(TTX_EINVAL, "ttx_cluster_entry: null argument");
    out[0] = out[1] = out[2] = 0;
    if (!h->cluster_nb()) return TTX_OK;
    const CreatePlan &s = h->sel;
    out[0] = (s.cl_powtab ? 1 : 0) | (s.cl_word ? 2 : 0) | (s.cl_lists ? 4 : 0);
    GroupState g0s;
    HIPCHECK(hipSetDevice(h->cfg.device));
    HIPCHECK(hipStreamSynchronize(h->stream));
    HIPCHECK(hipMemcpy(&g0s, h->P.gs, offsetof(GroupState, S), hipMemcpyDeviceToHost));
    out[1] = g0s.n_zload; out[2] = g0s.n_wload;
    return TTX_OK;
}
extern "C" int ttx_sweep_gap(const ttx_engine *h, int32_t out[4])
{
    if (!h || !out) return fail(TTX_EINVAL, "ttx_sweep_gap: null argument");
    const CreatePlan &s = h->sel;
    out[0] = (s.tail_event_kernel && !h->tail_event_retired) ? 1 : 0; out[1] = h->tail_event_fallbacks;
    out[2] = s.tail_lean ? 1 : 0; out[3] = s.cl_pack2 ? 1 : 0;
    return TTX_OK;
}
extern "C" int ttx_det_fallbacks(const ttx_engine *h) { return h ? h->det_fallbacks + h->de5_fallbacks : 0; }
extern "C" int ttx_fun_id(const ttx_engine *h) { return h ? h->cfg.fun_id : -1; }
extern "C" int ttx_set_profile(ttx_engine *h, int on) { if (!h) return fail(TTX_EINVAL, "null"); h->profile = on != 0; return TTX_OK; }
static void ct_plan(ttx_engine *h, const std::vector<char> &contracted, CtPlan &pl)
{
    ct_plan(h->d, h->n1.data() + 1, h->rfinal.data(), contracted, pl);
    for (int k = 0; k < h->d; k++) pl.cores[k].src = core_dev(h, k + 1);
}
static int ct_modesum(ttx_engine *h, const CtPlan &pl, const double *w, const CtCore *dcores, const CtTile *dtiles, OpTimer *tm)
{
    int rc;
    if ((rc = buf_reserve(h, SC_W, sizeof(double) * pl.wsize)) || (rc = buf_reserve(h, SC_M, sizeof(double) * std::max<size_t>(pl.msize, 1)))) return rc;
    std::vector<double> ones;
    if (!w) { ones.assign(pl.wsize, 1.0); w = ones.data(); }
    HIPCHECK(hipMemcpyAsync(buf<double>(h, SC_W), w, sizeof(double) * pl.wsize, hipMemcpyHostToDevice, h->stream));
    HIPCHECK(hipStreamSynchronize(h->stream));
    if (pl.tiles.empty()) return TTX_OK;
    if (tm && (rc = tm->start(h->stream))) return rc;
    hipLaunchKernelGGL(k_ct_modesum, dim3((unsigned)pl.tiles.size()), dim3(256), 0, h->stream, dcores, dtiles, h->RM, h->P.SS,
                       (const double *)buf<double>(h, SC_W), buf<double>(h, SC_M));
    return tm ? tm->stop(h->stream) : TTX_OK;
}
static int ct_finish(ttx_engine *h, const CtPlan &pl)
{
    HIPCHECK(hipStreamSynchronize(h->stream));
    HIPCHECK(hipGetLastError());
    h->ct = CtLast{0.0, pl.bytes};
    return pl.tiles.empty() ? TTX_OK : h->timer[TM_MODESUM].ms(&h->ct.ms);
}
static int ct_fill(ttx_engine *h, ttx_engine *e, const std::vector<int> &kept, const double *w)
{
    const int d = h->d, m = (int)kept.size();
    std::vector<char> contracted(d, 1);
    for (int k : kept) contracted[k] = 0;
    CtPlan pl;
    ct_plan(h, contracted, pl);
    const std::vector<int> &r = pl.r;
    std::vector<CtRun> runs;
    std::vector<int> run_left(m, -1);
    int run_trail = -1;
    size_t psize = 0, ssize = 0;
    for (int j = 0; j <= m; j++) {
        const int a = j ? kept[j - 1] + 1 : 0, b = (j < m ? kept[j] : d) - 1;
        if (b < a) continue;
        CtRun R{};
        R.k0 = a; R.cnt = b - a + 1; R.kind = j == 0 ? 0 : j == m ? 1 : 2; R.wmax = 1;
        for (int k = a; k <= b; k++) R.wmax = std::max(R.wmax, r[k + 1]);
        R.poff = psize; R.soff = ssize;
        psize += R.kind == 2 ? (size_t)r[a] * r[b + 1] : R.kind == 0 ? (size_t)r[b + 1] : (size_t)r[a];
        if (R.kind == 2 && 2 * (size_t)r[a] * R.wmax > TTX_CT_LDS) ssize += 2 * (size_t)r[a] * R.wmax;
        if (j < m) run_left[j] = (int)runs.size(); else run_trail = (int)runs.size();
        runs.push_back(R);
    }
    int rc;
    if ((rc = buf_reserve(h, SC_P, sizeof(double) * std::max<size_t>(psize, 1))) ||
        (rc = buf_reserve(h, SC_SCR, sizeof(double) * std::max<size_t>(ssize, 1)))) return rc;
    const double *Pb = buf<double>(h, SC_P);
    std::vector<CtKeep> keeps(m);
    long long items = 0;
    for (int j = 0; j < m; j++) {
        const int k = kept[j];
        CtKeep &K = keeps[j];
        K.src = pl.cores[k].src; K.dst = core_dev(e, j + 1);
        K.r0 = r[k]; K.n = h->n1[k + 1]; K.r1 = r[k + 1];
        K.P = run_left[j] >= 0 ? Pb + runs[run_left[j]].poff : nullptr;
        K.q0 = run_left[j] >= 0 ? r[runs[run_left[j]].k0] : K.r0;
        K.t = (j == m - 1 && run_trail >= 0) ? Pb + runs[run_trail].poff : nullptr;
        K.ncol = (K.n + 15) / 16; K.first = items; K.pad = 0;
        items += (long long)K.ncol * (K.t ? 1 : K.r1);
    }
    if (items > 0x7fffffffll) return fail(TTX_EINVAL, "ttx_contract: too many column tiles (%lld)", items);
    OpMeta meta(h->meta_host);
    const size_t o_cores = meta.put(pl.cores), o_tiles = meta.put(pl.tiles), o_runs = meta.put(runs), o_r = meta.put(r), o_moff = meta.put(pl.moff), o_keeps = meta.put(keeps);
// ... 2350 lines not shown
```

### ttcross_amd/csrc/ttx_init.h

```cpp
#pragma once
#include "ttx_integrands.h"
#include "ttx_wave.h"

struct DiagIdx { const int *n; int k, s; __device__ __forceinline__ int operator()(int p) const { return (k - 1 + s * (p - 1)) % n[p] + 1; } };
struct FixIdx { const int *ind; int self, selfval; __device__ __forceinline__ int operator()(int s) const { return s == self ? selfval : ind[s]; } };

template <int FUN>
__global__ __launch_bounds__(512) void k_init_samples(DevProb P, int snum, int nn, int ldsrows, int shift_hi)
{
    extern __shared__ __align__(16) double dyn[];
    double *par = dyn;
    __shared__ double sha[8], shv[8]; __shared__ int shi[8];
    const int g = blockIdx.x, tid = threadIdx.x;
    GroupState &gs = P.gs[g];
    for (int x = tid; x < P.npar; x += blockDim.x) par[x] = P.par[x];
    __syncthreads();
    double ba = -1.0, bv = 0.0; int bi = INT_MAX;
    const int m = P.d, VSr = ((m + 7) & ~7) + 8;
    short *rows = (short *)(((size_t)(dyn + P.npar) + 15) & ~(size_t)15);
    short *row = rows + (size_t)tid * VSr;
    if (FUN == FUN_ISING && P.arith && P.ising_id != 1 && ldsrows) {
        const int lane = tid & 63, wv = tid >> 6, nw = blockDim.x >> 6, n1m = P.n[1];
        double *xv = (double *)rows + (size_t)wv * 2 * (m + 64), *wvv = xv + (m + 64);
        int *nl = (int *)((double *)rows + (size_t)nw * 2 * (m + 64));
        for (int x = tid; x < m; x += blockDim.x) nl[x] = P.n[x + 1];
        __syncthreads();
        for (int il = wv; il < nn * snum; il += nw) {
            const int k = il % nn + 1, sft = il / nn;
            __builtin_amdgcn_wave_barrier();
            for (int x = lane; x < m; x += 64) { const int ix = (k - 1 + sft * x) % nl[x]; xv[x] = par[ix]; wvv[x] = par[n1m + ix]; }
            __builtin_amdgcn_wave_barrier();
            const double f = de_fast_point_wave(P.ising_id, m, xv, wvv, lane);
            const double a = fabs(f);
            if (lane == 0 && (a > ba || (a == ba && il < bi))) { ba = a; bv = f; bi = il; }
        }
    } else
    if (!ldsrows)
        for (int il = tid; il < nn * snum; il += blockDim.x) {
            DiagIdx ix{P.n, il % nn + 1, il / nn};
            double f = eval_fun<FUN>(P, par, ix, (long)g * P.HS + il);
            double a = fabs(f);
            if (a > ba || (a == ba && il < bi)) { ba = a; bv = f; bi = il; }
        }
    else {
    const int *nl = P.n + 1;
    if (ldsrows == 2) {
        int *nls = (int *)(((size_t)(rows + (size_t)blockDim.x * VSr) + 15) & ~(size_t)15);
        for (int x = tid; x < m; x += blockDim.x) nls[x] = P.n[x + 1];
        __syncthreads();
        nl = nls;
    }
    for (int il = tid; il < nn * snum; il += blockDim.x) {
        const int k = il % nn + 1, sft = il / nn;
        for (int p = 1; p <= m; p++) row[p - 1] = (short)((k - 1 + sft * (p - 1)) % nl[p - 1] + 1);
        for (int x = m; x < VSr; x++) row[x] = 1;
        row[m - 1 + 0] = row[m - 1];
        const int self = row[m - 1];
        row[m - 1] = 1;
        Src3 sx{row, m - 1, self, row + m};
        double f = eval_src3<FUN, true>(P, par, sx, (long)g * P.HS + il);
        double a = fabs(f);
        if (a > ba || (a == ba && il < bi)) { ba = a; bv = f; bi = il; }
    }
    }
    if (HOST_PASS1(FUN, P)) return;
    block_argmax(ba, bv, bi, sha, shv, shi);
    if (tid == 0) {
        gs.amax = ba;
        int gg = gs.gglobal;
        int lo = (int)((double)snum * (double)gg / P.nprocs);
        int hi = (gg + 1 == P.nprocs) ? snum : (int)((double)snum * (double)(gg + 1) / P.nprocs);
        gs.neval = (long long)nn * (hi - lo);
        if (g == 0) {
            if (bi == INT_MAX) bi = 0;
            int s = bi / nn, k = bi % nn + 1;
            for (int p = 1; p <= P.d; p++) P.ind0[p] = (k - 1 + s * (p - 1)) % P.n[p] + 1;
            P.ind0[P.d + 1] = 1;
        }
    }
}

template <int FUN>
__global__ __launch_bounds__(256) void k_init_fibers(DevProb P)
{
    extern __shared__ __align__(16) double dyn[];
// ... 70 lines not shown

__global__ __launch_bounds__(256) void k_init_final(DevProb P, int wave, double *out)
{
    __shared__ double dots[256], divs[256];
    const int g = blockIdx.x, tid = threadIdx.x;
    GroupState &gs = P.gs[g];
    const bool lastgroup = (gs.last + 1 == P.d && gs.gglobal == P.nprocs - 1);
    const int ncore = gs.last - gs.first + 1 + (lastgroup ? 1 : 0);
    double val = 1.0;
    if (P.has_quad) {
        for (int c0 = 0; c0 < ncore; c0 += 256) {
            if (wave) {
                const int lane = tid & 63, nw = blockDim.x >> 6, cend = min(ncore, c0 + 256);
                for (int c = c0 + (tid >> 6); c < cend; c += nw) {
                    const int p = gs.first + c, np_ = P.n[p];
                    const double *A = core_ptr(P, P.arg, g, p, gs.first), *w = P.quadw + (size_t)p * P.NM;
                    double t = 0.0;
                    for (int b = 0; b < np_; b += 64) {
                        const int j = b + lane, nb = min(64, np_ - b);
                        const double pr = j < np_ ? A[(size_t)P.RM * j] * w[j] : 0.0;
                        for (int k = 0; k < nb; k++) t = t + lane_get(pr, k);
                    }
                    if (lane == 0) dots[c - c0] = t;
                }
                if (c0 + tid < cend) { const int p = gs.first + c0 + tid; divs[tid] = p <= gs.last ? inv_ptr(P, g, p, gs.first)[0] : 0.0; }
            } else {
            const int c = c0 + tid;
            if (c < ncore) {
                const int p = gs.first + c;
                const double *A = core_ptr(P, P.arg, g, p, gs.first), *w = P.quadw + (size_t)p * P.NM;
                double t = 0.0;
                for (int j = 0; j < P.n[p]; j++) t = t + A[(size_t)P.RM * j] * w[j];
                dots[tid] = t;
            }
            }
            __syncthreads();
            if (tid == 0)
                for (int c2 = c0; c2 < min(ncore, c0 + 256); c2++) {
                    const int p = gs.first + c2;
                    if (p <= gs.last) val = val * dots[c2 - c0] / (wave ? divs[c2 - c0] : inv_ptr(P, g, p, gs.first)[0]);
                    else val = val * dots[c2 - c0];
                }
            __syncthreads();
        }
    }
    if (tid == 0) { gs.pivotmax_prev = gs.amax; gs.pivotmax = -1.0; gs.pivotmin = -1.0; gs.initval = val; }
    if (!out) return;
    const int m = P.d;
    const int *r = P.r + (size_t)g * (m + 2), *tp = P.tape + (size_t)g * (m + 2) * 4;
    for (int p = gs.first + tid; p <= gs.last; p += blockDim.x) {
        double *e = out + SUM_HDR + P.nprocs + 5 * p;
        e[0] = (double)r[p]; e[1] = (double)tp[4 * p]; e[2] = (double)tp[4 * p + 1]; e[3] = (double)tp[4 * p + 2]; e[4] = (double)tp[4 * p + 3];
    }
    if (g == 0)
        for (int p = tid; p <= m; p += blockDim.x)
            if (p < P.gs[0].first || p > P.gs[P.G - 1].last) { double *e = out + SUM_HDR + P.nprocs + 5 * p; for (int x = 0; x < 5; x++) e[x] = 0.0; }
    if (tid != 0) return;
    out[SUM_HDR + gs.gglobal] = val;
    if (gs.gglobal == 0) { out[SUM_AMAX] = gs.amax; out[SUM_PMAX] = -1.0; out[SUM_PMIN] = -1.0; }
    if (g != 0) return;
    double nev = 0.0, by = 0.0, nr = 0.0;
    for (int x = 0; x < P.G; x++) { const GroupState &o = P.gs[x]; nev += (double)o.neval; by += o.bytes_half; nr += (double)o.n_resid; }
    out[SUM_NEVAL] = nev; out[SUM_BYTES] = by; out[SUM_NRESID] = nr;
    out[SUM_VAL] = P.gs[0].val;
    for (int x = SUM_VAL + 1; x < SUM_HDR; x++) out[x] = 0.0;
}

__global__ __launch_bounds__(256) void k_reset(DevProb P, size_t SB, size_t QB)
{
    const size_t t0 = (size_t)blockIdx.x * blockDim.x + threadIdx.x, nt = (size_t)gridDim.x * blockDim.x;
    const size_t nr = (size_t)P.G * (P.d + 2);
    for (size_t x = t0; x < nr; x += nt) { P.r[x] = 1; P.rr[x] = 1; P.upd[x] = 0; }
    for (size_t x = t0; x < 4 * nr; x += nt) P.tape[x] = -1;
    for (size_t x = t0; x < SB; x += nt) P.sumsend[x] = 0.0;
    for (size_t x = t0; x < QB; x += nt) P.qsend[x] = 0.0;
    if (t0 < 4) P.ctl[t0] = 0;
    if (t0 < 2) P.strk[t0] = 0;
    if (P.lot_ctr) for (size_t x = t0; x < (size_t)P.G; x += nt) P.lot_ctr[x] = 0u;
    if (P.cl_ctr) {
        for (size_t x = t0; x < (size_t)P.G; x += nt) P.cl_ctr[x] = 0u;
        ClPart z; z.ab = 0.0; z.bb = 0.0; z.mx = 0.0; z.ix = 0; z.pad = 0;
        for (size_t x = t0; x < (size_t)2 * P.G * TTX_CLREC; x += nt) P.cl_part[x] = z;
    }
    for (size_t g = t0; g < (size_t)P.G; g += nt) {
        GroupState &gs = P.gs[g];
        gs.amax = 0.0; gs.pivotmax = -1.0; gs.pivotmin = -1.0; gs.pivotmax_prev = 0.0;
        gs.neval = 0; gs.rngpos = 0; gs.val = 0.0; gs.initval = 0.0; gs.bytes_half = 0.0; gs.n_resid = 0;
        gs.amax_bnd[0] = 0.0; gs.amax_bnd[1] = 0.0;
        gs.rngword = 0; gs.rngword_pos = 0; gs.zk_epoch = 0; gs.n_zload = 0; gs.n_wload = 0;
#ifdef TTX_STAMPS
        for (int a = 0; a < 2; a++) { gs.nstamp[a] = 0; for (int b = 0; b < 16; b++) gs.stamp[a][b] = 0; }
#endif
    }
}
```

### ttcross_amd/engine.py

```python
import ctypes
import os
import shutil
import subprocess
from ctypes import POINTER, c_char_p, c_double, c_int32, c_int64, c_uint8, c_uint64, c_void_p

import numpy as np

TTX_FUN_ISING, TTX_FUN_STDNORM, TTX_FUN_MVN, TTX_FUN_HOST = 1, 2, 3, 4
TTX_FUN_COSCOEFF = 5
TTX_FUN_DEVICE = 6
TTX_FUN_TRAINS = 7
TTX_FUN_PULLBACK = 8
TTX_PULLBACK_MAX = 8
TTX_TRAINS_MAX = 8
TTX_TOP_PRODUCT, TTX_TOP_RATIO, TTX_TOP_SQRTABS, TTX_TOP_DEVICE = 1, 2, 3, 4
TRAIN_OPS = {"product": TTX_TOP_PRODUCT, "ratio": TTX_TOP_RATIO, "sqrtabs": TTX_TOP_SQRTABS}
TTX_EVAL_EXACT, TTX_EVAL_MFMA, TTX_EVAL_AUTO = 0, 1, 2
EVAL_MODES = {"exact": TTX_EVAL_EXACT, "mfma": TTX_EVAL_MFMA, "auto": TTX_EVAL_AUTO}
TOPK_WHICH = {"abs": 0, "max": 1, "min": 2}
TTX_BASIS_COS, TTX_BASIS_LINEAR, TTX_BASIS_HALVE_FIRST = 1, 2, 1
BASIS_KINDS = {"cos": TTX_BASIS_COS, "linear": TTX_BASIS_LINEAR}
K_NAMES = ("lottery", "halfstep", "accept", "exchange", "quad", "other")

_HERE = os.path.dirname(os.path.abspath(__file__))
# ... 660 lines not shown
        pp = _dp(p) if p.size else None
        if fun is None:
            _check(L.ttx_set_integrand_pullback(self._h, len(layers), arr, refp, None, 0, None, pp, p.size))
        else:
            image_or_path, name = fun
            if isinstance(image_or_path, (bytes, bytearray, memoryview)):
                img = bytes(image_or_path)
                _check(L.ttx_set_integrand_pullback(self._h, len(layers), arr, refp, img, len(img), name.encode(), pp, p.size))
            else:
                _check(L.ttx_set_integrand_pullback_file(self._h, len(layers), arr, refp, os.fsencode(image_or_path), name.encode(), pp, p.size))
        self._operands = [y[0] for y in layers]
        return self

    def pullback_points(self, ind):
        ind = np.ascontiguousarray(ind, dtype=np.int32).reshape(-1, self.d)
        x, lq, v = np.zeros((ind.shape[0], self.d)), np.zeros(ind.shape[0]), np.zeros(ind.shape[0])
        _check(load_library().ttx_pullback_points(self._h, ind.shape[0], _ip(ind), _dp(x), _dp(lq), _dp(v)))
        return x, lq, v

    def pullback_last(self):
        ms, nl, ne, nf = c_double(), c_int64(), c_int64(), c_int64()
        _check(load_library().ttx_pullback_last(self._h, ctypes.byref(ms), ctypes.byref(nl), ctypes.byref(ne), ctypes.byref(nf)))
        return dict(ms=ms.value, launches=nl.value, elements=ne.value, failed=nf.value)

    def eval_device(self, ind):
        ind = np.ascontiguousarray(ind, dtype=np.int32).reshape(-1, self.d)
        out = np.zeros(ind.shape[0])
        _check(load_library().ttx_eval_device(self._h, ind.shape[0], _ip(ind), _dp(out)))
        return out

    @property
    def host_calls(self):
        return int(load_library().ttx_host_calls(self._h))

    @property
    def fun_id(self):
        L = load_library()
        L.ttx_fun_id.argtypes = [c_void_p]
        return L.ttx_fun_id(self._h)

    @property
    def arith(self):
        L = load_library()
        L.ttx_arith.argtypes = [c_void_p]
        return ("exact", "fast")[L.ttx_arith(self._h)]

    def sweep_path(self):
        L = load_library()
        L.ttx_sweep_path.argtypes = [c_void_p]
        return ("chain", "fused", "cluster")[L.ttx_sweep_path(self._h)]

    def plan(self):
        L = load_library()
        L.ttx_plan_describe.argtypes = [c_void_p, c_char_p, c_int64]
        buf = ctypes.create_string_buffer(1024)
        _check(L.ttx_plan_describe(self._h, buf, len(buf)))
        return dict(line.split(": ", 1) for line in buf.value.decode().splitlines())

    def cluster_eval(self):
        L = load_library()
        L.ttx_cluster_eval.argtypes = [c_void_p]
        return ("none", "predicated", "chunks", "closed")[L.ttx_cluster_eval(self._h)]

    @property
    def resid_halfsteps(self):
        L = load_library()
        L.ttx_resid_halfsteps.argtypes = [c_void_p]
        L.ttx_resid_halfsteps.restype = c_int64
        return int(L.ttx_resid_halfsteps(self._h))

    @property
    def cluster_fallbacks(self):
        L = load_library()
        L.ttx_cluster_fallbacks.argtypes = [c_void_p]
        return int(L.ttx_cluster_fallbacks(self._h))

    def cluster_entry(self):
        L = load_library()
        L.ttx_cluster_entry.argtypes = [c_void_p, ctypes.POINTER(c_int64)]
        out = (c_int64 * 3)()
        _check(L.ttx_cluster_entry(self._h, out))
        return {"powtab": bool(out[0] & 1), "word": bool(out[0] & 2), "lists": bool(out[0] & 4), "lists_taken": int(out[1]), "word_taken": int(out[2])}

    def sweep_gap(self):
        L = load_library()
        L.ttx_sweep_gap.argtypes = [c_void_p, ctypes.POINTER(ctypes.c_int32)]
        out = (ctypes.c_int32 * 4)()
        _check(L.ttx_sweep_gap(self._h, out))
        return {"tail_event": "kernel" if out[0] else "marker", "tail_event_fallbacks": int(out[1]), "tail_lean": bool(out[2]),
                "cl_pack2": bool(out[3])}

    @property
    def det_fallbacks(self):
        L = load_library()
        L.ttx_det_fallbacks.argtypes = [c_void_p]
        return int(L.ttx_det_fallbacks(self._h))

    def set_profile(self, on=True):
        _check(load_library().ttx_set_profile(self._h, 1 if on else 0))

    def run(self):
        _check(load_library().ttx_run(self._h))
        return self

    @property
    def neval(self):
        return int(load_library().ttx_neval(self._h))

    @property
    def seconds(self):
        return float(load_library().ttx_seconds(self._h))

    def sweeps(self):
        L = load_library()
        k = L.ttx_num_sweeps(self._h)
        buf = (SweepRec * k)()
        _check(L.ttx_get_sweeps(self._h, buf, k))
        return [dict(it=b.it, dir=b.dir, erank=b.erank, neval=b.neval, val=b.val, amax=b.amax,
                     pivotmax=b.pivotmax, pivotmin=b.pivotmin, seconds=b.seconds) for b in buf]

    def tapes(self):
        L = load_library()
        k = L.ttx_num_sweeps(self._h) - 1
        out = np.zeros((max(k, 0), self.d + 1, 4), dtype=np.int32)
        if k > 0:
            _check(L.ttx_get_tapes(self._h, _ip(out), out.size))
        return out

    def fast_tables(self, group, side=None, bond=None, cols=None):
        L = load_library()
        L.ttx_fast_tables.argtypes = [c_void_p, c_int32, c_int32, c_int32, c_int32, POINTER(c_int32), POINTER(c_int32)] + [POINTER(c_double)] * 3
        info = np.zeros(3, dtype=np.int32)
        if side is None:
            _check(L.ttx_fast_tables(self._h, group, 0, 0, 0, _ip(info), None, None, None, None))
            return int(info[1]), int(info[2])
        cols = 4096 if cols is None else int(cols)
        d = self.d
        idx = np.zeros(d * cols, dtype=np.int32)
        near, dv, piv = np.zeros((d + 1) * cols), np.zeros((d + 1) * cols), np.zeros(8 * cols)
        _check(L.ttx_fast_tables(self._h, group, side, bond, cols, _ip(info), _ip(idx), _dp(near), _dp(dv), _dp(piv)))
        r = int(info[0])
        ln = bond if side == 0 else d - bond
        return dict(r=r, idx=idx[:d * r].reshape(d, r)[:ln], near=near[:(d + 1) * r].reshape(d + 1, r), dv=dv[:(d + 1) * r].reshape(d + 1, r),
                    piv=piv[:8 * r].reshape(8, r))

    def ranks(self):
        r = np.zeros(self.d + 1, dtype=np.int32)
        _check(load_library().ttx_get_ranks(self._h, _ip(r)))
        return r

    def core(self, k):
        L = load_library()
        r = self.ranks()
        sz = L.ttx_core_size(self._h, k)
        buf = np.zeros(sz, dtype=np.float64)
        _check(L.ttx_get_core(self._h, k, _dp(buf)))
        return buf.reshape((r[k - 1], self._n[k - 1], r[k]), order="F")

    def _weights(self, w, who):
        if w is None:
            return None
        if len(w) != self.d or any(np.size(q) != int(nk) for q, nk in zip(w, self._n)):
            raise ValueError(f"{who}: {self.d} weight vectors of lengths {list(map(int, self._n))} expected")
        return np.ascontiguousarray(np.concatenate([np.asarray(q, dtype=np.float64).ravel() for q in w]))

    def quad(self, w=None):
# ... 951 lines not shown
```

Before: 256.0 million evals/s.

## Cache per-bond cluster node/weight tables in global images across sweeps

```diff
diff --git a/include/ttx.h b/include/ttx.h
--- a/include/ttx.h
+++ b/include/ttx.h
@@ -269,6 +269,7 @@
 int ttx_arith(const ttx_engine *h);
 int ttx_cluster_fallbacks(const ttx_engine *h);
 int ttx_cluster_entry(const ttx_engine *h, int64_t out[3]);
+int ttx_cluster_tables(const ttx_engine *h, int64_t out[4]);
 int ttx_sweep_gap(const ttx_engine *h, int32_t out[4]);
 int ttx_det_fallbacks(const ttx_engine *h);
 int ttx_fun_id(const ttx_engine *h);
diff --git a/ttcross_amd/csrc/ttx_addr.h b/ttcross_amd/csrc/ttx_addr.h
--- a/ttcross_amd/csrc/ttx_addr.h
+++ b/ttcross_amd/csrc/ttx_addr.h
@@ -1,6 +1,7 @@
 #pragma once
 #include <hip/hip_runtime.h>
 #include "ttx_dev.h"
+#include "ttx_cluster_rules.h"
 
 __device__ __forceinline__ double *core_ptr(const DevProb &P, double *base, int g, int p, int first)
 { return base + ((size_t)g * P.NC + (p - first)) * P.CS; }
@@ -12,3 +13,10 @@
 { return P.L + ((size_t)g * P.NC + (s - first + 1)) * (size_t)P.d * P.RM; }
 __device__ __forceinline__ short *R_ptr(const DevProb &P, int g, int s, int first)
 { return P.R + ((size_t)g * P.NC + (s - first)) * (size_t)P.d * P.RM; }
+__device__ __forceinline__ double *cl_timage(const DevProb &P, int g, int nsteps)
+{
+    return (double *)((int *)(P.cl_part + (size_t)2 * P.G * TTX_CLREC) + (size_t)P.G * cl_zimage_ints(nsteps, P.RM))
+           + (size_t)g * cl_img_group_doubles(nsteps, P.RM, cl_img_vs(P.d));
+}
+__device__ __forceinline__ int *cl_timage_rows(const DevProb &P, int g, int nsteps)
+{ return (int *)(cl_timage(P, g, nsteps) + cl_img_rows_at(nsteps, P.RM, cl_img_vs(P.d))); }
diff --git a/ttcross_amd/csrc/ttx_cluster.h b/ttcross_amd/csrc/ttx_cluster.h
--- a/ttcross_amd/csrc/ttx_cluster.h
+++ b/ttcross_amd/csrc/ttx_cluster.h
@@ -153,6 +153,33 @@
 __device__ __forceinline__ int *cl_zimage(const DevProb &P, int g, int nsteps)
 { return (int *)(P.cl_part + (size_t)2 * P.G * TTX_CLREC) + (size_t)g * cl_zimage_ints(nsteps, P.RM); }
 
+#define CL_IMG 32
+
+typedef double cl_d2 __attribute__((ext_vector_type(2)));
+template <int N>
+__device__ __forceinline__ void cl_tables_copy(const double *imgL, double *XL, int nL, int nR, unsigned Rb, int tid)
+{
+    const int ntot = nL + nR;
+#pragma unroll 1
+    for (int b0 = 0; b0 < ntot; b0 += N * CB) {
+        cl_d2 v[N]; unsigned a[N];
+#pragma unroll
+        for (int k = 0; k < N; k++)
+            if (b0 + k * CB < ntot) {
+                int x = b0 + k * CB + tid; x = x < ntot ? x : 0;
+                a[k] = x < nL ? 16u * (unsigned)x : 16u * (unsigned)(x - nL) + Rb;
+                v[k] = *(const cl_d2 *)((const char *)imgL + a[k]);
+            }
+#pragma unroll
+        for (int k = 0; k < N; k++)
+            if (b0 + k * CB < ntot) *(cl_d2 *)((char *)XL + a[k]) = v[k];
+    }
+}
+__device__ __forceinline__ void cl_table_out(double *img, const double *X, int rows, int RS, int tid)
+{
+    for (int x = tid; x < rows * (RS >> 1); x += CB) ((cl_d2 *)img)[x] = ((const cl_d2 *)X)[x];
+}
+
 template <bool CFAST, bool CPAD>
 __global__ __launch_bounds__(CB) void k_sweep_cluster(DevProb P, int dir, int nsteps, int NB, int ldsinv, int epoch, int zkeep)
 {
@@ -167,6 +194,7 @@
     constexpr int NFT = CFAST ? 64 : 1;
     __shared__ double fSL[NFT], fWL[NFT], fSR[NFT], fWR[NFT];
     __shared__ struct { int ii, jj, kk, qq, hcount, rc_k, rc_q, rr_i, rr_j; double pivot, amax, bytes_half; long long neval, n_resid; } s_rook;
+    __shared__ int s_tcnt[3];
     const int bid = blockIdx.x;
     const int g = (bid & 7) + 8 * (bid / (8 * NB)), cb = (bid >> 3) % NB;
     CSE_DECL;
@@ -276,6 +304,8 @@
     }
     const int bl0 = ptab ? (int)cl_powtab.v[lane] : (int)ttx_minstd_pow(2ull * lane);
     constexpr unsigned long long c64 = cl_minstd_pow_c(128);
+    double *const gimg = cl_timage(P, g, nsteps);
+    if (tid < 3) s_tcnt[tid] = 0;
     CSE(2);
     CST_DECL;
 
@@ -283,6 +313,8 @@
         if (pp > nbonds) break;
         const int p = (dir == 1) ? first + pp - 1 : last + 1 - pp;
         const int r0 = r[p - 1], r1 = r[p], r2 = r[p + 1], n1 = P.n[p], n2 = P.n[p + 1];
+        const int *const irow = (zkeep & CL_IMG) ? (const int *)(gimg + cl_img_rows_at(nsteps, RM, VS)) + 2 * (p - first) : r;
+        const int irL = irow[0], irR = irow[1];
         const int nlot = r0 + n1 + n2 + r2;
         double *Cp = core_ptr(P, P.col, g, p, first), *Wq = core_ptr(P, P.row, g, p + 1, first);
         double *Ap = core_ptr(P, P.arg, g, p, first), *Aq = core_ptr(P, P.arg, g, p + 1, first);
@@ -296,9 +328,30 @@
                 myns = P.cdf_ns[K]; sg_a0 = sp->a0; sg_al = sp->alast; sg_de = sp->delta; sg_k0 = sp->k0; sg_cn = sp->cnt;
             }
         };
+        const int AL = cl_img_used(p - 1, VS), AR = cl_img_used(m - p - 1, VS);
+        constexpr bool EARLY = CPAD || CFAST;
+        if (EARLY && (zkeep & CL_ZKEEP)) seg_issue(r0 * n1 - ZN[2 * (p - first)], n2 * r2 - ZN[2 * (p - first) + 1]);
+        double gl0 = 0.0, gl1 = 0.0, gu0 = 0.0, gu1 = 0.0;
+        if (EARLY && ldsinv) {
+            if (p > first) { const double *gL = inv_ptr(P, g, p - 1, first); if (tid < r0 * r0) gl0 = gL[tid]; if (tid + CB < r0 * r0) gl1 = gL[tid + CB]; }
+            if (p < last)  { const double *gU = inv_ptr(P, g, p + 1, first); if (tid < r2 * r2) gu0 = gU[tid]; if (tid + CB < r2 * r2) gu1 = gU[tid + CB]; }
+        }
+        bool cpL = false, cpR = false, outL = false, outR = false;
+        if (zkeep & CL_IMG) {
+            const int nL = __builtin_amdgcn_readfirstlane(irL), nR = __builtin_amdgcn_readfirstlane(irR);
+            cpL = AL > 0 && cl_img_valid(nL, r0); cpR = AR > 0 && cl_img_valid(nR, r2);
+            int tq = tid; asm volatile("" : "+v"(tq));
+            if (cpL || cpR)
+                cl_tables_copy<10>(gimg + cl_img_table_at(p - first, 0, RM, VS), XL, cpL ? r0 * (RS >> 1) : 0, cpR ? r2 * (RS >> 1) : 0, 8u * (unsigned)(RM * RS), tq);
+            const bool ownL = p > first || first == 1, ownR = p < last || last == m - 1;
+            if constexpr (EARLY) { outL = AL > 0 && !cpL && ownL; outR = AR > 0 && !cpR && ownR; }
+            if (tid == 0) {
+                if (AL > 0) { s_tcnt[cpL ? 0 : 1]++; if (!cpL && ownL && epoch > 1) s_tcnt[2]++; }
+                if (AR > 0) { s_tcnt[cpR ? 0 : 1]++; if (!cpR && ownR && epoch > 1) s_tcnt[2]++; }
+            }
+        }
         {
-            const int AL = min(VS, (p - 1 + 7) & ~7), AR = min(VS, (m - p - 1 + 7) & ~7);
-            if (AL > 0) {
+            if (AL > 0 && !cpL) {
                 int c = tid / AL, o = tid - c * AL;
                 const int dc = CB / AL, dO = CB - dc * AL;
                 while (c < r0) {
@@ -314,7 +367,7 @@
                     c += dc; o += dO; if (o >= AL) { o -= AL; c++; }
                 }
             }
-            if (AR > 0) {
+            if (AR > 0 && !cpR) {
                 int c = tid / AR, o = tid - c * AR;
                 const int dc = CB / AR, dO = CB - dc * AR;
                 while (c < r2) {
@@ -328,11 +381,21 @@
             }
         }
         if (ldsinv) {
-            if (p > first) { const double *gL = inv_ptr(P, g, p - 1, first); for (int x = tid; x < r0 * r0; x += CB) GL[x] = gL[x]; }
-            if (p < last)  { const double *gU = inv_ptr(P, g, p + 1, first); for (int x = tid; x < r2 * r2; x += CB) GU[x] = gU[x]; }
+            if (p > first) {
+                const double *gL = inv_ptr(P, g, p - 1, first);
+                if (EARLY && tid < r0 * r0) GL[tid] = gl0;
+                if (EARLY && tid + CB < r0 * r0) GL[tid + CB] = gl1;
+                for (int x = tid + (EARLY ? 2 * CB : 0); x < r0 * r0; x += CB) GL[x] = gL[x];
+            }
+            if (p < last) {
+                const double *gU = inv_ptr(P, g, p + 1, first);
+                if (EARLY && tid < r2 * r2) GU[tid] = gu0;
+                if (EARLY && tid + CB < r2 * r2) GU[tid + CB] = gu1;
+                for (int x = tid + (EARLY ? 2 * CB : 0); x < r2 * r2; x += CB) GU[x] = gU[x];
+            }
         }
         CST(0);
-        if (zkeep & CL_ZKEEP) seg_issue(r0 * n1 - ZN[2 * (p - first)], n2 * r2 - ZN[2 * (p - first) + 1]);
+        if (!EARLY && (zkeep & CL_ZKEEP)) seg_issue(r0 * n1 - ZN[2 * (p - first)], n2 * r2 - ZN[2 * (p - first) + 1]);
         static_assert(2 * (TTX_CLMAX + 1) <= 64 && TTX_CLMAX + TTX_CLMAX + 2 < 64, "the two slice rows and the shuffles of the fill fit one wave");
         if (wv == CB / 64 - 1) {
             const int side = lane > TTX_CLMAX ? 1 : 0, c = lane - side * (TTX_CLMAX + 1);
@@ -361,11 +424,14 @@
             if (sseg == 0) { if (sside) nsr = myns; else nsc = myns; }
         }
         if (tid < r0) {
-            double w = 1.0, wk = 1.0;
-            auto wstep = [&](double xv) { wk = wk * xv; w = w + wk; };
-            if constexpr (CPAD) chain8v<true>(XL + (size_t)tid * RS, p - 1, wstep);
-            else chain8v<false>(XL + (size_t)tid * RS, p - 1, wstep);
-            pLw[tid] = w; pLk[tid] = wk;
+            if (!cpL) {
+                double w = 1.0, wk = 1.0;
+                auto wstep = [&](double xv) { wk = wk * xv; w = w + wk; };
+                if constexpr (CPAD) chain8v<true>(XL + (size_t)tid * RS, p - 1, wstep);
+                else chain8v<false>(XL + (size_t)tid * RS, p - 1, wstep);
+                pLw[tid] = w; pLk[tid] = wk;
+                XL[(size_t)tid * RS + 2 * VS] = w; XL[(size_t)tid * RS + 2 * VS + 1] = wk;
+            } else { const cl_d2 st = *(const cl_d2 *)(XL + cl_img_state_at(tid, VS)); pLw[tid] = st.x; pLk[tid] = st.y; }
             if constexpr (CFAST) {
                 double sk = 1.0, ss = 0.0, ww = 1.0;
                 auto sstep = [&](double xv) { sk = sk * xv; ss = ss + sk; };
@@ -376,10 +442,13 @@
             }
         } else if (tid >= 64 && tid < 64 + r2) {
             const int c = tid - 64;
-            double v = 1.0, vk = 1.0;
-            auto vstep = [&](double xv) { vk = vk * xv; v = v + vk; };
-            chain8v<true>(XR + (size_t)c * RS, m - p - 1, vstep);
-            pRv[c] = v; pRk[c] = vk;
+            if (!cpR) {
+                double v = 1.0, vk = 1.0;
+                auto vstep = [&](double xv) { vk = vk * xv; v = v + vk; };
+                chain8v<true>(XR + (size_t)c * RS, m - p - 1, vstep);
+                pRv[c] = v; pRk[c] = vk;
+                XR[(size_t)c * RS + 2 * VS] = v; XR[(size_t)c * RS + 2 * VS + 1] = vk;
+            } else { const cl_d2 st = *(const cl_d2 *)(XR + cl_img_state_at(c, VS)); pRv[c] = st.x; pRk[c] = st.y; }
             if constexpr (CFAST) {
                 double sk = 1.0, ss = 0.0, ww = 1.0;
                 auto sstep = [&](double xv) { sk = sk * xv; ss = ss + sk; };
@@ -584,6 +653,14 @@
             rr_i = s_rook.rr_i; rr_j = s_rook.rr_j; pivot = s_rook.pivot; amax = s_rook.amax; bytes_half = s_rook.bytes_half; neval = s_rook.neval; n_resid = s_rook.n_resid;
         }
         CST(10);
+        if constexpr (!EARLY)
+            if ((zkeep & CL_IMG) && cb == 0) { outL = AL > 0 && !cpL && (p > first || first == 1); outR = AR > 0 && !cpR && (p < last || last == m - 1); }
+        if (cb == 0 && (outL || outR)) {
+            int *irow = (int *)(gimg + cl_img_rows_at(nsteps, RM, VS)) + 2 * (p - first);
+            int tq = tid; asm volatile("" : "+v"(tq));
+            if (outL) { cl_table_out(gimg + cl_img_table_at(p - first, 0, RM, VS), XL, r0, RS, tq); if (tid == 0) irow[0] = r0; }
+            if (outR) { cl_table_out(gimg + cl_img_table_at(p - first, 1, RM, VS), XR, r2, RS, tq); if (tid == 0) irow[1] = r2; }
+        }
         int *tape = P.tape + ((size_t)g * (m + 2) + p) * 4;
         const bool upd = accept_pivot(pivot, amax, pivotmax_prev, P.small_element, P.small_pivot);
         if (!upd) {
@@ -594,6 +671,12 @@
             const bool reuseA = (rc_k == kk && rc_q == qq), reuseB = (rr_i == ii && rr_j == jj);
             AppendTab tab{0, 0};
             if (cb == 0) tab = append_tables_fetch(P, g, p, first, ii, qq, tid);
+            const int cbL = EARLY ? NB - 1 : 0, cbR = EARLY ? NB - 1 : 1, wvR = EARLY ? 3 : 2;
+            const bool rowL = cb == cbL && wv == 2 && p < last, rowR = cb == cbR && wv == wvR && p > first && !rowL;
+            const bool trow = (zkeep & CL_IMG) && (rowL || rowR);
+            int *const tcnt = (int *)(gimg + cl_img_rows_at(nsteps, RM, VS)) + 2 * (p - first) + (rowL ? 2 : -1);
+            int trows = 0;
+            if (trow) trows = *tcnt;
             if (reuseA && reuseB) {
                 if (cb == 0)
                     for (int s = tid; s < r1; s += CB) {
@@ -677,6 +760,23 @@
                     if (lane == 0) { kl[pos] = key; ZN[2 * b + wv] = nl + 1; }
                 }
             }
+            if (trow && __builtin_amdgcn_readfirstlane(trows) == r1) {
+                const bool left = rowL;
+                const int len = left ? p - 1 : m - p - 1, An = cl_img_used(len + 1, VS), nd = left ? jj : kk;
+                const double *prow = left ? XL + (size_t)(ii - 1) * RS : XR + (size_t)(qq - 1) * RS;
+                double *dst = gimg + cl_img_table_at(p - first + (left ? 1 : -1), left ? 0 : 1, RM, VS) + (size_t)r1 * RS;
+                const double xn = par[nd - 1], wn = par[n1m + nd - 1], tn = CPAD ? 0.0 : par[0], tw = CPAD ? 1.0 : par[n1m];
+                int lq = lane; asm volatile("" : "+v"(lq));
+                for (int o = lq; o < An; o += 64) {
+                    dst[o] = cl_img_new_entry(!left || CPAD, o, len, xn, tn, [&](int t) { return prow[t]; });
+                    dst[VS + o] = cl_img_new_entry(!left, o, len, wn, tw, [&](int t) { return prow[VS + t]; });
+                }
+                if (lane == 0) {
+                    const ClState st = cl_state_step(left ? ClState{pLw[ii - 1], pLk[ii - 1]} : ClState{pRv[qq - 1], pRk[qq - 1]}, xn);
+                    dst[2 * VS] = st.s; dst[2 * VS + 1] = st.k;
+                    *tcnt = r1 + 1;
+                }
+            }
             pivot_range(pivotmax, pivotmin, fabs(pivot));
         }
         CST(14);
@@ -705,6 +805,7 @@
             gs.bytes_half = bytes_half; gs.n_resid = n_resid;
             if (K->zkeep & CL_WORD) { gs.rngword = sA0; gs.rngword_pos = rngpos; }
             if (K->zkeep & CL_ZCARRY) gs.zk_epoch = K->epoch;
+            if (K->zkeep & CL_IMG) { gs.n_tcopy += s_tcnt[0]; gs.n_tgather += s_tcnt[1]; gs.n_tgather_own += s_tcnt[2]; }
             if (P.tail_side) gs.amax_bnd[epoch & 1] = 0.0;
         }
         __syncthreads();
diff --git a/ttcross_amd/csrc/ttx_cluster_rules.h b/ttcross_amd/csrc/ttx_cluster_rules.h
--- a/ttcross_amd/csrc/ttx_cluster_rules.h
+++ b/ttcross_amd/csrc/ttx_cluster_rules.h
@@ -81,3 +81,23 @@
 #define CL_PACK_LEFT 1
 TTX_HD int cl_pack_block(int part, int NB, bool split) { return (part == CL_PACK_LEFT && split && NB >= 2) ? 1 : 0; }
 TTX_HD size_t cl_zimage_ints(int nsteps, int RM) { return ((size_t)nsteps * 2 * (size_t)RM + 2 * (size_t)nsteps + 3) & ~(size_t)3; }
+
+TTX_HD int cl_img_vs(int m) { return ((m + 7) & ~7) + 8; }
+TTX_HD int cl_img_rs(int VS) { return 2 * VS + 2; }
+TTX_HD int cl_img_used(int len, int VS) { const int a = (len + 7) & ~7; return a < VS ? a : VS; }
+TTX_HD size_t cl_img_table_doubles(int RM, int VS) { return (size_t)RM * (size_t)cl_img_rs(VS); }
+TTX_HD size_t cl_img_table_at(int b, int side, int RM, int VS) { return ((size_t)b * 2 + (size_t)side) * cl_img_table_doubles(RM, VS); }
+TTX_HD size_t cl_img_rows_at(int nsteps, int RM, int VS) { return (size_t)nsteps * 2 * cl_img_table_doubles(RM, VS); }
+TTX_HD size_t cl_img_group_doubles(int nsteps, int RM, int VS) { return cl_img_rows_at(nsteps, RM, VS) + (((size_t)nsteps + 1) & ~(size_t)1); }
+TTX_HD size_t cl_img_node_at(int row, int o, int VS) { return (size_t)row * cl_img_rs(VS) + o; }
+TTX_HD size_t cl_img_weight_at(int row, int o, int VS) { return (size_t)row * cl_img_rs(VS) + VS + o; }
+TTX_HD size_t cl_img_state_at(int row, int VS) { return (size_t)row * cl_img_rs(VS) + 2 * VS; }
+TTX_HD bool cl_img_valid(int rows, int rank) { return rows > 0 && rows == rank; }
+struct ClState { double s, k; };
+TTX_HD ClState cl_state_step(ClState a, double x) { const double k = a.k * x; return ClState{a.s + k, k}; }
+template <class PAR>
+TTX_HD double cl_img_new_entry(bool front, int o, int len, double xnew, double tail, PAR par)
+{
+    if (front) return o == 0 ? xnew : (o <= len ? par(o - 1) : tail);
+    return o < len ? par(o) : (o == len ? xnew : tail);
+}
diff --git a/ttcross_amd/csrc/ttx_create_plan.h b/ttcross_amd/csrc/ttx_create_plan.h
--- a/ttcross_amd/csrc/ttx_create_plan.h
+++ b/ttcross_amd/csrc/ttx_create_plan.h
@@ -13,6 +13,7 @@
 #include "../../include/ttx.h"
 #include "ttx_dev.h"
 #include "ttx_qr_plan.h"
+#include "ttx_cluster_rules.h"
 
 #if defined(__HIPCC__)
 #define TTX_PLAN_HD __host__ __device__ inline
@@ -68,6 +69,7 @@
     EnvText tail_event;
     bool tail_lean_off = false;
     bool cl_pack2_off = false;
+    bool cl_img_off = false;
 };
 template <class Get>
 CreateEnv create_env_from(Get get)
@@ -100,7 +102,7 @@
     v.init_wide_off = off("TTX_INIT_WIDE"); v.quad_lds_off = off("TTX_QUAD_LDS");
     v.cl_powtab_off = off("TTX_CL_POWTAB"); v.cl_word_off = off("TTX_CL_WORD"); v.cl_lists_off = off("TTX_CL_LISTS");
     v.tail_event = text("TTX_TAIL_EVENT"); v.tail_lean_off = off("TTX_TAIL_LEAN");
-    v.cl_pack2_off = off("TTX_CL_PACK2");
+    v.cl_pack2_off = off("TTX_CL_PACK2"); v.cl_img_off = off("TTX_CL_IMG");
     return v;
 }
 struct DevCaps { int ncu = 0; bool coop = false; };
@@ -148,6 +150,7 @@
     int cluster_var = 0;
     int cluster_ldsinv = 0, cluster_zkeep = 0, cluster_coop = 0;
     bool cl_powtab = true, cl_word = true, cl_lists = false;
+    bool cl_img = false; size_t cl_img_bytes = 0;
     int cl_test_abort = 0; bool dbg_waves = false;
     bool sweep_tail = true;
     bool sweep_tail_side = true;
@@ -353,6 +356,7 @@
         const size_t zk = sizeof(int) * ((size_t)p.nbmax * 2 * RM + 2 * p.nbmax + 4);
         if (p.lds_cluster + zk <= TTX_LDS_WORK) { p.cluster_zkeep = 1; p.lds_cluster += zk; }
         p.cl_powtab = !env.cl_powtab_off; p.cl_word = !env.cl_word_off; p.cl_lists = p.cluster_zkeep && !env.cl_lists_off;
+        p.cl_img = !env.cl_img_off;
         const bool cfastc = p.want_fast && fun == TTX_FUN_ISING && p.ising_id == 1;
         if (env.cl_pad.set && env.cl_pad.v != "0" && env.cl_pad.v != "1") return plan_refuse(p, TTX_EINVAL, "TTX_CL_PAD must be 0 or 1 (got %s)", env.cl_pad.v.c_str());
         p.cluster_var = cfastc ? 2 : (unit && !(env.cl_pad.set && env.cl_pad.v == "0")) ? 1 : 0;
@@ -414,4 +418,6 @@
     else if (p.sweep_want == SWEEP_FUSED) { if (p.fused_ok) p.fused = 1; }
     else if (p.sweep_want == SWEEP_AUTO) { if (cluster_ok) p.cluster = p.cluster_cand; else if (p.fused_ok && p.G == 1) p.fused = 1; }
     if (p.cluster && p.cluster_var == 2) p.arith = 1;
-}
+    if (!p.cluster) p.cl_img = false;
+    p.cl_img_bytes = p.cl_img ? sizeof(double) * (size_t)p.G * cl_img_group_doubles(p.nbmax, p.RM, cl_img_vs(p.d)) : 0;
+}
diff --git a/ttcross_amd/csrc/ttx_dev.h b/ttcross_amd/csrc/ttx_dev.h
--- a/ttcross_amd/csrc/ttx_dev.h
+++ b/ttcross_amd/csrc/ttx_dev.h
@@ -47,7 +47,8 @@
     long long n_resid;
     double amax_bnd[2];
     unsigned long long rngword, rngword_pos;
-    int zk_epoch, n_zload, n_wload, pad1;
+    int zk_epoch, n_zload, n_wload;
+    int n_tcopy, n_tgather, n_tgather_own, pad1, pad2;
 #ifdef TTX_STAMPS
     long long stamp[2][16]; long long nstamp[2];
 #endif
@@ -130,6 +131,7 @@
     unsigned *cl_ctr;
     int *cl_abort;
     int cl_test_abort;
+    int cl_img;
     struct ClPart *cl_part;
     long long *dbg;
 };
diff --git a/ttcross_amd/csrc/ttx_engine.hip b/ttcross_amd/csrc/ttx_engine.hip
--- a/ttcross_amd/csrc/ttx_engine.hip
+++ b/ttcross_amd/csrc/ttx_engine.hip
@@ -567,8 +567,9 @@
     if (s.cluster) {
         unsigned *ctr; ClPart *cp;
         A_(dev_alloc(h, &ctr, G));
-        A_(dev_alloc(h, &cp, 2 * G * TTX_CLREC + (s.cl_lists ? (G * cl_zimage_ints(s.nbmax, s.RM) * sizeof(int) + sizeof(ClPart) - 1) / sizeof(ClPart) : 0)));
-        P.cl_ctr = ctr; P.cl_part = cp;
+        const size_t zbytes = (s.cl_lists || s.cl_img) ? G * cl_zimage_ints(s.nbmax, s.RM) * sizeof(int) : 0;
+        A_(dev_alloc(h, &cp, 2 * G * TTX_CLREC + (zbytes + s.cl_img_bytes + sizeof(ClPart) - 1) / sizeof(ClPart)));
+        P.cl_ctr = ctr; P.cl_part = cp; P.cl_img = s.cl_img ? 1 : 0;
 #ifdef TTX_STAMPS
         if (s.dbg_waves) { long long *dbg; A_(dev_alloc(h, &dbg, (size_t)8 * 64 * 8)); P.dbg = dbg; }
 #endif
@@ -1344,7 +1345,8 @@
         const CreatePlan &s = h->sel;
         int dir = 2 - it_ % 2, epoch = it_, nsteps = h->nbmax, NB = s.cluster, ldsinv = s.cluster_ldsinv;
         int zkeep = (s.cluster_zkeep ? CL_ZKEEP : 0) | (s.cl_lists ? CL_ZCARRY : 0) | (s.cl_word ? CL_WORD : 0) | (s.cl_powtab ? CL_POWTAB : 0)
-                    | (s.cl_pack2 ? CL_PACK2 : 0);
+                    | (s.cl_pack2 ? CL_PACK2 : 0)
+                    | (s.cl_img ? CL_IMG : 0);
         const dim3 grid(8 * NB * ((G + 7) / 8)), block(CB);
         KScope ks(h, TTX_K_HALFSTEP, 1);
         if (!cluster) hipLaunchKernelGGL(k_sweep_fused, dim3(G), dim3(FB), s.lds_fused, st, P, dir, nsteps);
@@ -2826,6 +2828,21 @@
     HIPCHECK(hipStreamSynchronize(h->stream));
     HIPCHECK(hipMemcpy(&g0s, h->P.gs, offsetof(GroupState, S), hipMemcpyDeviceToHost));
     out[1] = g0s.n_zload; out[2] = g0s.n_wload;
+    return TTX_OK;
+}
+extern "C" int ttx_cluster_tables(const ttx_engine *h, int64_t out[4])
+{
+    if (!h || !out) return fail(TTX_EINVAL, "ttx_cluster_tables: null argument");
+    out[0] = out[1] = out[2] = out[3] = 0;
+    if (!h->cluster_nb()) return TTX_OK;
+    out[0] = h->sel.cl_img ? 1 : 0;
+    HIPCHECK(hipSetDevice(h->cfg.device));
+    HIPCHECK(hipStreamSynchronize(h->stream));
+    for (int g = 0; g < h->P.G; g++) {
+        GroupState gs;
+        HIPCHECK(hipMemcpy(&gs, h->P.gs + g, offsetof(GroupState, S), hipMemcpyDeviceToHost));
+        out[1] += gs.n_tcopy; out[2] += gs.n_tgather; out[3] += gs.n_tgather_own;
+    }
     return TTX_OK;
 }
 extern "C" int ttx_sweep_gap(const ttx_engine *h, int32_t out[4])
diff --git a/ttcross_amd/csrc/ttx_init.h b/ttcross_amd/csrc/ttx_init.h
--- a/ttcross_amd/csrc/ttx_init.h
+++ b/ttcross_amd/csrc/ttx_init.h
@@ -1,6 +1,7 @@
 #pragma once
 #include "ttx_integrands.h"
 #include "ttx_wave.h"
+#include "ttx_addr.h"
 
 struct DiagIdx { const int *n; int k, s; __device__ __forceinline__ int operator()(int p) const { return (k - 1 + s * (p - 1)) % n[p] + 1; } };
 struct FixIdx { const int *ind; int self, selfval; __device__ __forceinline__ int operator()(int s) const { return s == self ? selfval : ind[s]; } };
@@ -237,12 +238,17 @@
         ClPart z; z.ab = 0.0; z.bb = 0.0; z.mx = 0.0; z.ix = 0; z.pad = 0;
         for (size_t x = t0; x < (size_t)2 * P.G * TTX_CLREC; x += nt) P.cl_part[x] = z;
     }
+    if (P.cl_img) {
+        const int nsteps = P.NC - 1;
+        for (size_t x = t0; x < (size_t)P.G * 2 * nsteps; x += nt) cl_timage_rows(P, (int)(x / (2 * nsteps)), nsteps)[x % (2 * nsteps)] = 0;
+    }
     for (size_t g = t0; g < (size_t)P.G; g += nt) {
         GroupState &gs = P.gs[g];
         gs.amax = 0.0; gs.pivotmax = -1.0; gs.pivotmin = -1.0; gs.pivotmax_prev = 0.0;
         gs.neval = 0; gs.rngpos = 0; gs.val = 0.0; gs.initval = 0.0; gs.bytes_half = 0.0; gs.n_resid = 0;
         gs.amax_bnd[0] = 0.0; gs.amax_bnd[1] = 0.0;
         gs.rngword = 0; gs.rngword_pos = 0; gs.zk_epoch = 0; gs.n_zload = 0; gs.n_wload = 0;
+        gs.n_tcopy = 0; gs.n_tgather = 0; gs.n_tgather_own = 0;
 #ifdef TTX_STAMPS
         for (int a = 0; a < 2; a++) { gs.nstamp[a] = 0; for (int b = 0; b < 16; b++) gs.stamp[a][b] = 0; }
 #endif
diff --git a/ttcross_amd/engine.py b/ttcross_amd/engine.py
--- a/ttcross_amd/engine.py
+++ b/ttcross_amd/engine.py
@@ -766,6 +766,13 @@
         _check(L.ttx_cluster_entry(self._h, out))
         return {"powtab": bool(out[0] & 1), "word": bool(out[0] & 2), "lists": bool(out[0] & 4), "lists_taken": int(out[1]), "word_taken": int(out[2])}
 
+    def cluster_tables(self):
+        L = load_library()
+        L.ttx_cluster_tables.argtypes = [c_void_p, ctypes.POINTER(c_int64)]
+        out = (c_int64 * 4)()
+        _check(L.ttx_cluster_tables(self._h, out))
+        return {"images": bool(out[0]), "copies": int(out[1]), "gathers": int(out[2]), "own_gathers_late": int(out[3])}
+
     def sweep_gap(self):
         L = load_library()
         L.ttx_sweep_gap.argtypes = [c_void_p, ctypes.POINTER(ctypes.c_int32)]
```

Measured after the change: 256.7 million evals/s (median of 2 runs). No clear change (+0.3%).
